# mwhoffman/pybo

Hardware: AMD Instinct MI355X
Metric: BO-step wall-clock (GP fit + 1e6-candidate acq sweep) at N obs; steps/sec (higher is better)
Workload: dtype f64

## Files before the change

pybo_amd/_lib.py:

```python
import ctypes as C
import os

import numpy as np



def hw_queues_hint():
    try:
        q = int(os.environ.get('GPU_MAX_HW_QUEUES', '4'))
    except ValueError:
        q = 4
    if q >= 8:
        return None
    return ('pybo_amd: several device handles on GPU_MAX_HW_QUEUES=%d hardware queues; export GPU_MAX_HW_QUEUES=8 before '
            'the HIP runtime starts to keep their streams apart (see INTEGRATION.md)' % q)


_HERE = os.path.dirname(os.path.abspath(__file__))
LIB_PATH = os.environ.get('GPX_LIB_PATH') or os.path.join(
    _HERE, 'csrc', 'libgpx_diag.so' if os.environ.get('GPX_DIAGNOSTICS', '0') not in ('', '0') else 'libgpx.so')

_P = C.c_void_p
_D = C.POINTER(C.c_double)
_I = C.POINTER(C.c_int64)
# ... 558 lines not shown
        ti = np.empty(k, dtype=np.int64)
        out = np.empty(M) if want_all else None
        mu = np.empty(M) if want_moments else None
        s2 = np.empty(M) if want_moments else None
        self._check(self._lib.gpx_sweep_update(self._h, aid, _ptr(params), nparams, k, _ptr(tv) if k else None,
                                               _ptr(ti) if k else None, _ptr(out), _ptr(mu), _ptr(s2)))
        return dict(top_val=tv, top_idx=ti, acq=out, mu=mu, s2=s2)

    def sweep_cache_size(self):
        return int(self._lib.gpx_sweep_cache_size(self._h))

    def sweep_batch(self, kind, param, nb, want_s2_all=False):
        aid = acq_id(kind)
        params, nparams = _acq_params(param)
        n = max(int(nb), 0)
        out = dict(sel_val=np.empty(n), sel_idx=np.empty(n, dtype=np.int64), sel_s2=np.empty(n))
        if want_s2_all:
            out['s2_all'] = np.empty(self.sweep_cache_size())
        self._check(self._lib.gpx_sweep_batch(self._h, aid, _ptr(params), nparams, int(nb), _ptr(out['sel_val']), _ptr(out['sel_idx']),
                                              _ptr(out['sel_s2']), _ptr(out.get('s2_all'))))
        return out

    def sweep_dev(self, acq, param, dXc_ptr, M, k, d_acq=None, d_mu=None, d_s2=None):
        aid = acq_id(acq)
        params, nparams = _acq_params(param)
        tv = np.empty(k)
        ti = np.empty(k, dtype=np.int64)
        self._check(self._lib.gpx_sweep_dev(self._h, aid, _ptr(params), nparams, _P(dXc_ptr), M, k,
                                            _ptr(tv) if k else None, _ptr(ti) if k else None,
                                            _P(d_acq) if d_acq else None, _P(d_mu) if d_mu else None,
                                            _P(d_s2) if d_s2 else None))
        return tv, ti

    @staticmethod
    def ensemble_sweep(engines, acq, param, Xc, k=0, want_all=True, want_moments=False):
        lead = engines[0]
        handles = (_P * len(engines))(*[e._h for e in engines])
        aid = acq_id(acq)
        params, nparams = _acq_params(param)
        tv = np.empty(k)
        ti = np.empty(k, dtype=np.int64)
        if isinstance(Xc, DeviceGrid):
            M = len(Xc)
            lead._check(lead._lib.gpx_ensemble_sweep_dev(handles, len(engines), aid, _ptr(params), nparams, Xc.ptr, M,
                                                         k, _ptr(tv) if k else None, _ptr(ti) if k else None,
                                                         None, None, None))
            return dict(top_val=tv, top_idx=ti, acq=None, mu=None, s2=None)
        Xc = _f64(Xc).reshape(-1, lead.d)
        M = len(Xc)
        out = np.empty(M) if want_all else None
        mu = np.empty(M) if want_moments else None
        s2 = np.empty(M) if want_moments else None
        lead._check(lead._lib.gpx_ensemble_sweep(handles, len(engines), aid, _ptr(params), nparams, _ptr(Xc), M, k,
                                                 _ptr(tv) if k else None, _ptr(ti) if k else None, _ptr(out),
                                                 _ptr(mu), _ptr(s2)))
        return dict(top_val=tv, top_idx=ti, acq=out, mu=mu, s2=s2)

    @staticmethod
    def ensemble_batch(engines, kind, param, nb):
        lead = engines[0]
        handles = (_P * len(engines))(*[e._h for e in engines])
        aid = acq_id(kind)
        params, nparams = _acq_params(param)
        n = max(int(nb), 0)
        out = dict(sel_val=np.empty(n), sel_idx=np.empty(n, dtype=np.int64), sel_s2=np.empty((len(engines), n)))
        lead._check(lead._lib.gpx_ensemble_sweep_batch(handles, len(engines), aid, _ptr(params), nparams, int(nb), _ptr(out['sel_val']),
                                                       _ptr(out['sel_idx']), _ptr(out['sel_s2'])))
        return out

    @staticmethod
    def ensemble_predict(engines, Xc):
        lead = engines[0]
        handles = (_P * len(engines))(*[e._h for e in engines])
        Xc = _f64(Xc).reshape(-1, lead.d)
        n, M, d = len(engines), len(Xc), lead.d
        mu, s2 = np.empty((n, M)), np.empty((n, M))
        dmu, ds2 = np.empty((n, M, d)), np.empty((n, M, d))
        lead._check(lead._lib.gpx_ensemble_predict(handles, n, _ptr(Xc), M, _ptr(mu), _ptr(s2), _ptr(dmu), _ptr(ds2)))
        return mu, s2, dmu, ds2

    def rff_gram(self, W, b):
        W = _f64(W)
        b = _f64(b)
        n = len(b)
        A = np.empty((n, n))
        v = np.empty(n)
        self._check(self._lib.gpx_rff_gram(self._h, _ptr(W), _ptr(b), n, _ptr(A), _ptr(v)))
        return A, v

    def rff_gram_batch(self, W, b):
        W = _f64(W)
        S, n, d = W.shape
        b = _f64(b).reshape(S, n)
        A = np.empty((S, n, n))
        v = np.empty((S, n))
        self._check(self._lib.gpx_rff_gram_batch(self._h, _ptr(W), _ptr(b), S, n, _ptr(A), _ptr(v)))
        return A, v

    def rff_posterior(self, W, b, z, sc):
        W = _f64(W)
        S, n, d = W.shape
        b = _f64(b).reshape(S, n)
        z = _f64(z).reshape(S, n)
        theta = np.empty((S, n))
        self._check(self._lib.gpx_rff_posterior(self._h, _ptr(W), _ptr(b), _ptr(z), S, n, float(sc), _ptr(theta)))
        return theta

    def rff_sweep(self, W, b, theta, bias, Xc, k=0, want_all=True):
        W = _f64(W)
        S, n, d = W.shape
        b = _f64(b).reshape(S, n)
        theta = _f64(theta).reshape(S, n)
        Xc = _f64(Xc).reshape(-1, d)
        M = len(Xc)
        tv = np.empty((S, k))
        ti = np.empty((S, k), dtype=np.int64)
        out = np.empty((S, M)) if want_all else None
        self._check(self._lib.gpx_rff_sweep(self._h, _ptr(W), _ptr(b), _ptr(theta), S, n, d, bias, _ptr(Xc), M,
                                            k, _ptr(tv) if k else None, _ptr(ti) if k else None, _ptr(out)))
        return dict(top_val=tv, top_idx=ti, vals=out)

    def rff_eval_grad(self, W, b, theta, bias, Xc):
        W = _f64(W)
        n, d = W.shape
        b = _f64(b)
        theta = _f64(theta)
        Xc = _f64(Xc).reshape(-1, d)
        M = len(Xc)
        f = np.empty(M)
        g = np.empty((M, d))
        self._check(self._lib.gpx_rff_grad(self._h, _ptr(W), _ptr(b), _ptr(theta), n, d, bias, _ptr(Xc), M,
                                           _ptr(f), _ptr(g)))
        return f, g

    def rff_sweep_dev(self, W, b, theta, bias, dXc_ptr, M, k):
        W = _f64(W)
        S, n, d = W.shape
        b = _f64(b).reshape(S, n)
        theta = _f64(theta).reshape(S, n)
        tv = np.empty((S, k))
        ti = np.empty((S, k), dtype=np.int64)
        self._check(self._lib.gpx_rff_sweep_dev(self._h, _ptr(W), _ptr(b), _ptr(theta), S, n, d, bias,
                                                _P(dXc_ptr), M, k, _ptr(tv), _ptr(ti), None))
        return tv, ti

    def timers(self, reset=False):
        out = np.zeros(len(TIMER_NAMES))
        self._lib.gpx_timers(self._h, _ptr(out), len(out), 1 if reset else 0)
        return dict(zip(TIMER_NAMES, out.tolist()))

    PRUNE_PATHS = ('plain', 'gate declined', 'pruned', 'fell back')

    def prune_report(self, vectors=True):
        scal = np.full(20, np.nan)
        self._check(self._lib.gpx_prune_report(self._h, _ptr(scal), len(scal), None, None, 0, None, None, 0))
        names = ('path', 'M', 'k', 'G', 'Gg', 'done', 'cap', 'nsurv', 'S', 'delta', 'tau', 'gate_s2', 'thr_key', 'kept',
                 'bound_kernel', 'guard', 'nR', 'nsurv2', 'E', 'gate_hint')
        r = dict(zip(names, scal.tolist()))
        r['gate_hint'] = r['gate_hint'] == 1.0
        r['bound_kernel'] = None if np.isnan(r['bound_kernel']) else ('generic', 'mfma', 'mfma32')[int(r['bound_kernel'])]
        for n in ('path', 'M', 'k', 'G', 'Gg', 'done', 'cap', 'nsurv', 'kept', 'nR', 'nsurv2'):
            r[n] = int(r[n])
        r['path'] = self.PRUNE_PATHS[r['path']]
        if vectors and r['path'] in ('pruned', 'fell back'):
            M = r['M']
            nidx = r['nsurv'] if r['path'] == 'pruned' else 0
            r['ub'] = np.empty(M)
            r['idx'] = np.empty(nidx, dtype=np.int64)
            kept = bool(r['kept'])
            r['ub_kept'] = np.empty(M) if kept else None
            r['seed_idx'] = np.empty(r['G'], dtype=np.int64) if kept else None
            self._check(self._lib.gpx_prune_report(self._h, _ptr(scal), len(scal), _ptr(r['ub']), _ptr(r['idx']), nidx,
                                                   _ptr(r['ub_kept']), _ptr(r['seed_idx']), r['G'] if kept else 0))
            if r['nR'] > 0 and kept:
                r['ub2'] = np.empty(nidx)
                r['idx2'] = np.empty(r['nsurv2'], dtype=np.int64)
                r['qR'] = np.empty(nidx)
                self._check(self._lib.gpx_prune_rows(self._h, _ptr(r['qR']), _ptr(r['ub2']), _ptr(r['idx2']), r['nsurv2']))
        return r

    @staticmethod
    def ensemble_prune_report(engines, vectors=True):
        lead = engines[0]
        handles = (_P * len(engines))(*[e._h for e in engines])
        scal = np.full(11 + len(engines), np.nan)
        lead._check(lead._lib.gpx_ensemble_prune_report(handles, len(engines), _ptr(scal), len(scal), None, None, 0))
        names = ('path', 'M', 'k', 'G', 'Gg', 'done', 'cap', 'nsurv', 'tau', 'gate')
        r = dict(zip(names, scal[:10].tolist()))
        for n in names[:8]:
            r[n] = int(r[n])
        r['path'] = Engine.PRUNE_PATHS[r['path']]
        r['delta'] = scal[10:10 + len(engines)].copy()
        r['gate_hint'] = scal[10 + len(engines)] == 1.0
        if vectors and r['path'] in ('pruned', 'fell back'):
            nidx = r['nsurv'] if r['path'] == 'pruned' else 0
            r['ub'] = np.empty(r['M'])
            r['idx'] = np.empty(nidx, dtype=np.int64)
            lead._check(lead._lib.gpx_ensemble_prune_report(handles, len(engines), _ptr(scal), len(scal), _ptr(r['ub']), _ptr(r['idx']),
                                                            nidx))
        return r

    def prune_dots(self):
        M = self.prune_report(vectors=False)['M']
        out = np.empty(M)
        self._check(self._lib.gpx_prune_dots(self._h, _ptr(out)))
        return out

    def chol_trace(self, nblocks, full_log=False):
        out = np.zeros(20 * nblocks + 8 * 1024 + 16 + (4 << 20 if full_log else 0), dtype=np.int64)
        n = self._lib.gpx_chol_trace(self._h, _ptr(out), out.size)
        if n < 20 * nblocks:
            return None
        self.last_chol_profile = out[20 * nblocks:20 * nblocks + 8192].reshape(1024, 8).copy()
        self.last_chol_tasklog = None
        if full_log and n >= out.size:
            self.last_chol_tasklog = out[20 * nblocks + 8192 + 16:].reshape(1024, 1024, 4).copy()
        out = out[:20 * nblocks]
        t0 = out[0]
        self.last_chol_trace_origin = int(t0)
        diag = (out[:4 * nblocks].reshape(nblocks, 4)[:, :3] - t0) / 100.0
        crit = out[4 * nblocks:].reshape(nblocks, 8, 2).astype(np.float64)
        crit = np.where(crit > 0, (crit - t0) / 100.0, np.nan)
        return diag, crit

    def sync(self):
        self._check(self._lib.gpx_sync(self._h))
```

pybo_amd/csrc/api.hip:

```cpp
#include <math.h>
#include <stdio.h>
#include <stdlib.h>
#include <string.h>

#include <algorithm>
#include <cmath>
#include <functional>
#include <new>

#include "gpx_internal.h"
#include "gpx_diag.h"
#include "mes_math.h"
#include "kg_math.h"

using namespace gpx;

static thread_local std::string g_create_err;

#define HIPCHK(h, call)                                                                     \
    do {                                                                                    \
        hipError_t e_ = (call);                                                             \
        if (e_ != hipSuccess) {                                                             \
            char buf_[512];                                                                 \
            snprintf(buf_, sizeof buf_, "%s failed: %s (%s:%d)", #call, hipGetErrorString(e_), \
                     __FILE__, __LINE__);                                                   \
            (h)->err = buf_;                                                                \
            return (e_ == hipErrorOutOfMemory) ? GPX_EOOM : GPX_EHIP;                       \
        }                                                                                   \
    } while (0)

static int fail(gpx_handle* h, int code, const char* msg) {
    h->err = msg;
    return code;
}

template <typename F>
static int guarded(gpx_handle* h, F&& body) noexcept {
    try {
        return body();
    } catch (const std::bad_alloc&) {
        if (h) {
            try { h->err = "out of host memory"; } catch (...) {}
        }
        return GPX_EOOM;
    } catch (...) {
        if (h) {
            try { h->err = "unexpected C++ exception inside libgpx"; } catch (...) {}
        }
        return GPX_EHIP;
    }
}

template <typename T>
static int ensure(gpx_handle* h, T*& p, int64_t& cap, int64_t need) {
    if (need <= cap && p) return GPX_OK;
    if (p) HIPCHK(h, hipFree(p));
    p = nullptr;
    cap = 0;
    HIPCHK(h, hipMalloc((void**)&p, (size_t)need * sizeof(T)));
    cap = need;
    return GPX_OK;
}

static hipEvent_t ev_get(gpx_handle* h) {
    if (!h->pool.empty()) {
        hipEvent_t e = h->pool.back();
        h->pool.pop_back();
        return e;
    }
    hipEvent_t e = nullptr;
    hipEventCreate(&e);
    return e;
}
static void harvest_finished(gpx_handle* h) {
    size_t keep = 0;
    for (size_t i = 0; i < h->pending.size(); ++i) {
        EventPair p = h->pending[i];
        if (hipEventQuery(p.b) == hipSuccess) {
            float ms = 0.f;
            if (hipEventElapsedTime(&ms, p.a, p.b) == hipSuccess) h->tacc[p.slot] += ms;
            h->pool.push_back(p.a);
            h->pool.push_back(p.b);
        } else {
            h->pending[keep++] = p;
        }
    }
    h->pending.resize(keep);
}

struct Span {
    gpx_handle* h;
    EventPair p;
    Span(gpx_handle* h_, int slot) : h(h_) {
        if (h->pending.size() >= 256) harvest_finished(h);
        p.a = ev_get(h);
        p.b = ev_get(h);
        p.slot = slot;
        hipEventRecord(p.a, h->stream);
    }
    ~Span() {
        hipEventRecord(p.b, h->stream);
        h->pending.push_back(p);
    }
};
static void harvest(gpx_handle* h) {
    hipStreamSynchronize(h->stream);
    if (h->spec_launched && h->stream3) hipStreamSynchronize(h->stream3);
    for (auto& p : h->pending) {
        float ms = 0.f;
        if (hipEventElapsedTime(&ms, p.a, p.b) == hipSuccess) h->tacc[p.slot] += ms;
        h->pool.push_back(p.a);
        h->pool.push_back(p.b);
    }
    h->pending.clear();
}

enum { SHIP = 0, DIAG = 1 };
struct Option {
    const char* name;
    int diag;
    int64_t lo, hi;
    const char* bad;
    void (*set)(gpx_handle* h, int64_t v);
    bool (*ok)(int64_t v) = nullptr;
    const char* bad_ok = nullptr;
};
template <int gpx_handle::*F>
static void store(gpx_handle* h, int64_t v) { h->*F = (int)v; }
static bool mult128(int64_t v) { return v % 128 == 0; }
static const int64_t BIG = INT64_MAX;
static const char* const TG = "chol_tg*: out of range";
static const char* const TRTRI = "trtri_ahead*: out of range";
static const char* const XBG = "x_bg*: out of range";
static const Option kOptions[] = {
    {"chunk", SHIP, 128, BIG, "chunk must be a positive multiple of 128", [](gpx_handle* h, int64_t v) { h->chunk = v; }, mult128},
    {"super_m", SHIP, 1, 16, "super_m must be 1, 2, 4, 8 or 16", store<&gpx_handle::super_m>, [](int64_t v) { return (v & (v - 1)) == 0; }},
    {"tile_order", SHIP, -1, 31, "tile_order: -1 (by size) or bits 0-1 tile map (0..3), bits 2-4 k-loop schedule (1 .. 7)",
     store<&gpx_handle::tile_order>, [](int64_t v) { return v == -1 || v >= 4; }},
    {"sweep_cache", SHIP, -1, 1, "sweep_cache must be 1, 0 or -1",
     [](gpx_handle* h, int64_t v) { h->cache_on = (v == 1); if (v < 0) { h->cache_valid = false; h->npend = 0; } }},
    {"prune", SHIP, -1, 1, "prune must be -1 (by size and gate), 0 (never) or 1 (wherever legal)", store<&gpx_handle::prune>},
    {"prune_keep", DIAG, 0, 1, "prune_keep must be 0 or 1", store<&gpx_handle::prune_keep>},
    {"prune_bound", DIAG, -1, 2, "prune_bound must be -1 (by guard), 0 (generic kernel), 1 (matrix-pipe kernel) or 2 (fp32 matrix-pipe kernel)", store<&gpx_handle::prune_bound>},
    {"prune_rows", DIAG, -1, 1000000, "prune_rows must be -1 (by size), 0 (no second bound) or a number of block rows", store<&gpx_handle::prune_rows>},
    {"short_map", DIAG, -1, 1, "short_map must be -1 (by size), 0 (never) or 1 (wherever tile map 3 is in use)", store<&gpx_handle::short_map>},
    {"chol_w", SHIP, 0, 8, "chol_w must be 0 (by size) or in [2, 8]", store<&gpx_handle::chol_w>, [](int64_t v) { return v != 1; }},
    {"chol_tg", SHIP, -1, 1000000000, TG, store<&gpx_handle::chol_tg>, [](int64_t v) { return v == 0 || v == 1; }, "chol_tg must be 0 or 1"},
    {"chol_tg_chunks", DIAG, -1, 1000000000, TG, store<&gpx_handle::tg_chunks>},
    {"chol_tg_grid", DIAG, -1, 1000000000, TG, store<&gpx_handle::tg_grid>},
    {"chol_tg_trace", DIAG, -1, 1000000000, TG, store<&gpx_handle::tg_trace>},
    {"chol_tg_isolate", DIAG, -1, 1000000000, TG, store<&gpx_handle::tg_isolate>},
    {"chol_tg_nap", DIAG, -1, 1000000000, TG, [](gpx_handle* h, int64_t v) { h->tg_nap = (int)std::max<int64_t>(0, std::min<int64_t>(127, v)); }},
    {"chol_tg_tmo_ms", SHIP, -1, 1000000000, TG, store<&gpx_handle::tg_tmo_ms>},
    {"chol_tg_min", SHIP, -1, 1000000000, TG, [](gpx_handle* h, int64_t v) { h->tg_min = (int)std::max<int64_t>(1, v); }},
    {"chol_tg_max", SHIP, -1, 1000000000, TG, [](gpx_handle* h, int64_t v) { h->tg_max = (int)std::max<int64_t>(1, v); }},
    {"chol_tg_db", SHIP, -1, 1000000000, TG, [](gpx_handle* h, int64_t v) { h->tg_db = (v < 0) ? -1 : (v != 0 ? 1 : 0); }},
    {"chol_tg_db_max", SHIP, -1, 1000000000, TG, [](gpx_handle* h, int64_t v) { h->tg_db_max = (int)std::max<int64_t>(0, v); }},
    {"chol_tg_fuse", SHIP, -1, 1000000000, TG, [](gpx_handle* h, int64_t v) { h->tg_fuse = (v != 0) ? 1 : 0; }},
    {"trtri_ahead", SHIP, 0, 1000000, TRTRI, [](gpx_handle* h, int64_t v) { h->trtri_ahead = (v != 0) ? 1 : 0; }},
    {"trtri_ahead_min", SHIP, 0, 1000000, TRTRI, [](gpx_handle* h, int64_t v) { h->trtri_ahead_min = (int)std::max<int64_t>(4, v); }},
    {"chol_fuse", SHIP, 0, 1, "chol_fuse must be 0 or 1", store<&gpx_handle::chol_fuse>},
    {"chol_graph", SHIP, 0, 1, "chol_graph must be 0 or 1", store<&gpx_handle::chol_graph>},
    {"chol_merge", SHIP, 0, 100000, "chol_merge: 0 (off) or a minimum number of block rows", store<&gpx_handle::chol_merge>},
    {"chol_rl", SHIP, 0, 1, "chol_rl must be 0 or 1", store<&gpx_handle::chol_rl>},
    {"x_skip", DIAG, 0, 7, "x_skip: bits 0..2", store<&gpx_handle::x_skip>},
    {"x_bg", DIAG, 0, 10000000, XBG, store<&gpx_handle::x_bg>},
    {"x_bg_lds", DIAG, 0, 10000000, XBG, store<&gpx_handle::x_bg_lds>},
    {"x_bg_iters", DIAG, 0, 10000000, XBG, store<&gpx_handle::x_bg_iters>},
    {"x_rff", DIAG, 0, 1, "x_rff must be 0 (by size) or 1 (the round-3 kernel)", [](gpx_handle*, int64_t v) { gpx::g_rff_variant = (int)v; }},
    {"grad_form", SHIP, 0, 2, "grad_form must be 0 (auto), 1 (two passes) or 2 (one pass)", store<&gpx_handle::grad_form>},
    {"grad_rb_cs", DIAG, 0, 65536, "grad_rb_cs must be a multiple of 128 (0 = default)", store<&gpx_handle::grad_rb_cs>, mult128},
    {"grad_kernel", SHIP, -1, 1, "grad_kernel must be -1 (auto), 0 or 1", store<&gpx_handle::grad_kernel>},
    {"trtri_left", SHIP, 0, 1, "trtri_left must be 0 or 1", store<&gpx_handle::trtri_left>},
    {"refine_inverse", SHIP, 0, 1, "refine_inverse must be 0 or 1", [](gpx_handle* h, int64_t v) { h->refine_inverse = (v != 0); }},
    {"eager_inverse", SHIP, 0, 1, "eager_inverse must be 0 or 1", [](gpx_handle* h, int64_t v) { h->eager_inverse = (v != 0); }},
};

extern "C" int gpx_set_option(gpx_handle* h, const char* name, int64_t value) {
    return guarded(h, [&]() -> int {
        if (!h) return GPX_EARG;
        h->prune_hint = h->ens_hint = PruneHint();
        if (!name) return GPX_EARG;
        for (const Option& o : kOptions) {
            if (strcmp(name, o.name)) continue;
            if (o.diag && !gpx_diagnostics())
                return fail(h, GPX_EARG, "diagnostic option: only in a library built with -DGPX_DIAGNOSTICS (libgpx_diag.so)");
            if (value < o.lo || value > o.hi) return fail(h, GPX_EARG, o.bad);
            if (o.ok && !o.ok(value)) return fail(h, GPX_EARG, o.bad_ok ? o.bad_ok : o.bad);
            o.set(h, value);
            return GPX_OK;
        }
        return fail(h, GPX_EARG, "unknown option");
    });
}

static std::string apply_env_options(gpx_handle* h) {
    const char* env = getenv("GPX_OPTIONS");
    const std::string all(env ? env : "");
    for (size_t pos = 0; pos < all.size();) {
        size_t end = all.find(',', pos);
        if (end == std::string::npos) end = all.size();
        const std::string kv = all.substr(pos, end - pos);
        pos = end + 1;
        if (kv.empty()) continue;
        const size_t eq = kv.find('=');
        char* tail = nullptr;
        const long long v = (eq == std::string::npos) ? 0 : strtoll(kv.c_str() + eq + 1, &tail, 10);
        if (eq == std::string::npos || eq == 0 || !tail || *tail != 0 || tail == kv.c_str() + eq + 1 ||
            gpx_set_option(h, kv.substr(0, eq).c_str(), (int64_t)v) != GPX_OK)
            return kv;
    }
    return "";
}

extern "C" int gpx_version(void) { return 680; }

extern "C" const char* gpx_last_error(const gpx_handle* h) {
    return h ? h->err.c_str() : g_create_err.c_str();
}

static int create_impl(int device, void* stream, gpx_handle** out);

extern "C" int gpx_create(int device, void* stream, gpx_handle** out) {
    try {
        return create_impl(device, stream, out);
    } catch (...) {
        if (out) *out = nullptr;
        return GPX_EOOM;
    }
}

static int create_impl(int device, void* stream, gpx_handle** out) {
    if (!out) { g_create_err = "gpx_create: out is NULL"; return GPX_EARG; }
    *out = nullptr;
    int ndev = 0;
    hipError_t e = hipGetDeviceCount(&ndev);
    if (e != hipSuccess || ndev <= 0) {
        g_create_err = std::string("gpx_create: no HIP device (") + hipGetErrorString(e) + ")";
        return GPX_EHIP;
    }
    if (device < 0 || device >= ndev) { g_create_err = "gpx_create: bad device index"; return GPX_EARG; }
    gpx_handle* h = new (std::nothrow) gpx_handle();
    if (!h) { g_create_err = "gpx_create: out of host memory"; return GPX_EOOM; }
    h->device = device;
    if ((e = hipSetDevice(device)) != hipSuccess) {
        g_create_err = std::string("hipSetDevice: ") + hipGetErrorString(e);
        delete h;
        return GPX_EHIP;
    }
    if (stream) {
        h->stream = (hipStream_t)stream;
    } else {
        if ((e = hipStreamCreateWithFlags(&h->stream, hipStreamNonBlocking)) != hipSuccess) {
            g_create_err = std::string("hipStreamCreate: ") + hipGetErrorString(e);
            delete h;
            return GPX_EHIP;
        }
        h->own_stream = true;
    }
    if (hipMalloc((void**)&h->dsmall, 64 + 16 * 8 + DMAX * 8 + 32) != hipSuccess) {
        g_create_err = "gpx_create: device allocation failed";
        delete h;
        return GPX_EOOM;
    }
    if (hipHostMalloc((void**)&h->hinv, (size_t)DMAX * 8, hipHostMallocDefault) != hipSuccess ||
        hipEventCreateWithFlags(&h->ev_inv, hipEventDisableTiming) != hipSuccess) {
        g_create_err = "gpx_create: pinned host allocation failed";
        hipFree(h->dsmall);
        delete h;
        return GPX_EOOM;
    }
    h->dflag = reinterpret_cast<int*>(h->dsmall);
    h->dscal = reinterpret_cast<double*>(h->dsmall + 64);
    h->dinvell = h->dscal + 16;
    h->dclk = reinterpret_cast<unsigned long long*>(h->dinvell + DMAX);
    (void)hipMemsetAsync(h->dclk, 0, 32, h->stream);
    (void)hipStreamSynchronize(h->stream);
    *out = h;
    const std::string bad = apply_env_options(h);
    if (!bad.empty()) {
        g_create_err = "gpx_create: GPX_OPTIONS: bad entry '" + bad + "'";
        *out = nullptr;
        gpx_destroy(h);
        return GPX_EARG;
    }
    return GPX_OK;
}

int gpx::ensure_side_streams(gpx_handle* h) {
    if (h->stream2) return GPX_OK;
    int prio_lo = 0, prio_hi = 0;
    hipDeviceGetStreamPriorityRange(&prio_lo, &prio_hi);
    bool ok_ev = true;
    for (auto& e : h->ev_row) ok_ev = ok_ev && hipEventCreateWithFlags(&e, hipEventDisableTiming) == hipSuccess;
    if (!ok_ev || hipStreamCreateWithPriority(&h->stream2, hipStreamNonBlocking, prio_lo) != hipSuccess ||
        hipStreamCreateWithFlags(&h->stream3, hipStreamNonBlocking) != hipSuccess ||
        hipStreamCreateWithPriority(&h->stream4, hipStreamNonBlocking, prio_lo) != hipSuccess ||
        hipEventCreateWithFlags(&h->ev_chain, hipEventDisableTiming) != hipSuccess ||
        hipEventCreateWithFlags(&h->ev_far, hipEventDisableTiming) != hipSuccess ||
        hipEventCreateWithFlags(&h->ev_rest, hipEventDisableTiming) != hipSuccess)
        return fail(h, GPX_EHIP, "side stream / event creation failed");
    return GPX_OK;
}

extern "C" int gpx_destroy(gpx_handle* h) {
    if (!h) return GPX_OK;
    hipSetDevice(h->device);
    hipStreamSynchronize(h->stream);
    if (h->ahead_top != 0 && h->stream2) { hipStreamSynchronize(h->stream2); h->ahead_top = 0; }
    tg_free(h);
    for (auto& p : h->pending) { hipEventDestroy(p.a); hipEventDestroy(p.b); }
    for (auto e : h->pool) hipEventDestroy(e);
    void* ptrs[] = {h->dXs, h->dXraw, h->dy, h->dS, h->dR, h->dT, h->dU, h->da, h->dalpha, h->dsmall, h->dKs, h->dQp, h->dXc, h->dout, h->dblkv, h->dblki,
                    h->dtopv, h->drff, h->drffs, h->dgrad, h->dens, h->dprune, h->dkeep, h->dcZ, h->dcq, h->dbatch, h->dhyper, h->dpend, h->drefine, h->dspec, h->dbsel, h->djoint, h->dkg, h->dkgw};
    for (void* p : ptrs)
        if (p) hipFree(p);
    if (h->hpin) hipHostFree(h->hpin);
    if (h->hinv) hipHostFree(h->hinv);
    if (h->chol_exec) hipGraphExecDestroy(h->chol_exec);
    if (h->ev_inv) hipEventDestroy(h->ev_inv);
    if (h->ev_spec_go) hipEventDestroy(h->ev_spec_go);
    if (h->ev_spec_done) hipEventDestroy(h->ev_spec_done);
    if (h->stream_bg) { hipStreamSynchronize(h->stream_bg); hipStreamDestroy(h->stream_bg); }
    if (h->stream2) { hipStreamSynchronize(h->stream2); hipStreamDestroy(h->stream2); }
    if (h->stream3) { hipStreamSynchronize(h->stream3); hipStreamDestroy(h->stream3); }
    if (h->stream4) { hipStreamSynchronize(h->stream4); hipStreamDestroy(h->stream4); }
    if (h->ev_rest) hipEventDestroy(h->ev_rest);
    for (auto e : h->ev_row)
        if (e) hipEventDestroy(e);
    if (h->ev_chain) hipEventDestroy(h->ev_chain);
    if (h->ev_far) hipEventDestroy(h->ev_far);
    if (h->own_stream) hipStreamDestroy(h->stream);
    delete h;
    return GPX_OK;
}


extern "C" int gpx_sync(gpx_handle* h) {
    return guarded(h, [&]() -> int {
        if (!h) return GPX_EARG;
        HIPCHK(h, hipStreamSynchronize(h->stream));
        return GPX_OK;
    });
}

extern "C" int64_t gpx_chol_tasks2(int nblocks, int chunks, int16_t* out, int64_t cap, int64_t* counts) {
    if (!counts) return -1;
    try {
        return gpx::tg_tasks_copy(nblocks, chunks, out, cap, counts);
    } catch (...) {
        return -1;
    }
}

extern "C" int64_t gpx_chol_trace(gpx_handle* h, int64_t* out, int64_t n) {
    if (!h || !out || n <= 0) return 0;
    if (hipSetDevice(h->device) != hipSuccess || hipStreamSynchronize(h->stream) != hipSuccess) return 0;
    static_assert(sizeof(long long) == sizeof(int64_t), "trace words");
    return tg_trace_copy(h, reinterpret_cast<long long*>(out), n);
}

static void report_head(const gpx_handle::SelectRecord& r, double* out) {
    const double head[8] = {(double)r.path, (double)r.M, (double)r.k, (double)r.G, (double)r.Gg, (double)r.done, (double)r.cap, (double)r.nsurv};
    std::copy(head, head + 8, out);
}
static int report_vectors(gpx_handle* h, const gpx_handle::SelectRecord& r, double* ub, int64_t* idx, int64_t cap_idx) {
    if (ub) HIPCHK(h, hipMemcpy(ub, r.ub, (size_t)r.M * 8, hipMemcpyDeviceToHost));
    const int64_t nidx = std::min(std::min(r.nsurv, r.cap), cap_idx);
    if (idx && nidx > 0) HIPCHK(h, hipMemcpy(idx, r.idx, (size_t)nidx * 8, hipMemcpyDeviceToHost));
    return GPX_OK;
}

extern "C" int gpx_prune_report(gpx_handle* h, double* scal, int nscal, double* ub, int64_t* idx, int64_t cap_idx,
                                double* ub_kept, int64_t* seed_idx, int64_t cap_seed) {
    return guarded(h, [&]() -> int {
        if (!h) return GPX_EARG;
        if (!scal || nscal < 0) return fail(h, GPX_EARG, "prune_report: NULL output");
        const gpx_handle::PruneRecord& r = h->prune_rec;
        if (r.path < 0) return fail(h, GPX_ESTATE, "prune_report: no sweep has completed its argument checks since the record was last cleared");
        const bool bound = r.path >= 2;
        if ((ub || idx || ub_kept || seed_idx) && !bound)
            return fail(h, GPX_ESTATE, "prune_report: the last sweep did not reach its bound pass");
        if ((ub_kept || seed_idx) && !r.kept)
            return fail(h, GPX_ESTATE, "prune_report: the last sweep ran without the option prune_keep");
        HIPCHK(h, hipSetDevice(h->device));
        HIPCHK(h, hipStreamSynchronize(h->stream));
        double sc[16];
        int st[4] = {0, 0, 0, 0};
        for (double& v : sc) v = NAN;
        if (bound) {
            HIPCHK(h, hipMemcpy(sc, r.sc, sizeof sc, hipMemcpyDeviceToHost));
            HIPCHK(h, hipMemcpy(st, r.st, sizeof st, hipMemcpyDeviceToHost));
        }
        const bool guarded_bound = bound && r.bound_kernel < 0;
        double out[20];
        report_head(r, out);
        const double tail[12] = {sc[0], sc[1], sc[5], r.gate, bound ? (double)st[2] : NAN, r.kept ? 1.0 : 0.0,
                                 bound ? (guarded_bound ? sc[9] + sc[12] : 0.0) : NAN, guarded_bound ? sc[8] : NAN,
                                 (double)r.nR, (double)r.nsurv2, guarded_bound ? sc[10] : NAN, r.hinted ? 1.0 : 0.0};
        std::copy(tail, tail + 12, out + 8);
        for (int i = 0; i < nscal && i < 20; ++i) scal[i] = out[i];
        int rc;
        if ((rc = report_vectors(h, r, ub, idx, cap_idx))) return rc;
        if (ub_kept) HIPCHK(h, hipMemcpy(ub_kept, h->dkeep, (size_t)r.M * 8, hipMemcpyDeviceToHost));
        const int64_t nseed = std::min(r.G, cap_seed);
        if (seed_idx && nseed > 0)
            HIPCHK(h, hipMemcpy(seed_idx, h->dkeep + r.M * 8, (size_t)nseed * 8, hipMemcpyDeviceToHost));
        return GPX_OK;
    });
}

extern "C" int gpx_prune_rows(gpx_handle* h, double* qR, double* ub2, int64_t* idx2, int64_t cap_idx2) {
    return guarded(h, [&]() -> int {
        if (!h) return GPX_EARG;
        const gpx_handle::PruneRecord& r = h->prune_rec;
        if (r.path != 2 || r.nR <= 0) return fail(h, GPX_ESTATE, "prune_rows: the last sweep ran no second bound");
        if (!r.kept) return fail(h, GPX_ESTATE, "prune_rows: the last sweep ran without the option prune_keep");
        HIPCHK(h, hipSetDevice(h->device));
        HIPCHK(h, hipStreamSynchronize(h->stream));
        if (qR) HIPCHK(h, hipMemcpy(qR, r.qR, (size_t)r.nsurv * 8, hipMemcpyDeviceToHost));
        if (ub2) HIPCHK(h, hipMemcpy(ub2, r.ub2, (size_t)r.nsurv * 8, hipMemcpyDeviceToHost));
        const int64_t n2 = std::min(r.nsurv2, cap_idx2);
        if (idx2 && n2 > 0) HIPCHK(h, hipMemcpy(idx2, r.idx2, (size_t)n2 * 8, hipMemcpyDeviceToHost));
        return GPX_OK;
    });
}

extern "C" int gpx_prune_dots(gpx_handle* h, double* dots) {
    return guarded(h, [&]() -> int {
        if (!h) return GPX_EARG;
        if (!dots) return fail(h, GPX_EARG, "prune_dots: NULL output");
        const gpx_handle::PruneRecord& r = h->prune_rec;
        if (r.path < 2 || !r.kept) return fail(h, GPX_ESTATE, "prune_dots: the last sweep kept no bound pass (option prune_keep)");
        HIPCHK(h, hipSetDevice(h->device));
        HIPCHK(h, hipStreamSynchronize(h->stream));
        HIPCHK(h, hipMemcpy(dots, h->dkeep + (r.M + r.G) * 8, (size_t)r.M * 8, hipMemcpyDeviceToHost));
        return GPX_OK;
    });
}

extern "C" int gpx_timers(gpx_handle* h, double* out, int n, int reset) {
    return guarded(h, [&]() -> int {
        if (!h) return GPX_EARG;
        if (!out || n < 0) return fail(h, GPX_EARG, "timers: NULL output");
        harvest(h);
        unsigned long long clk[4] = {0, 0, 0, 0};
        (void)hipMemcpyAsync(clk, h->dclk, 32, hipMemcpyDeviceToHost, h->stream);
        (void)hipStreamSynchronize(h->stream);
        h->tacc[T_SCLK] = clk[1] ? 100.0 * (double)clk[0] / (double)clk[1] : 0.0;
        h->tacc[T_RFFCLK] = clk[3] ? 100.0 * (double)clk[2] / (double)clk[3] : 0.0;
        const int m = std::min(n, (int)T_COUNT);
        for (int i = 0; i < m; ++i) out[i] = h->tacc[i];
        if (reset) {
            for (int i = 0; i < T_COUNT; ++i) h->tacc[i] = 0;
            (void)hipMemsetAsync(h->dclk, 0, 32, h->stream);
        }
        return m;
    });
}

static void spec_cancel(gpx_handle* h) {
    if (h->spec_launched && h->ev_spec_done) hipStreamWaitEvent(h->stream, h->ev_spec_done, 0);
    h->spec_active = false;
    h->spec_launched = false;
    h->apply_pending = false;
}

static int check_fit_args(gpx_handle* h, const void* X, int64_t N, int64_t d, const void* y, int kid,
                          const double* ell, double rho, double sn2) {
    if (!h) return GPX_EARG;
    if (!X || !y || !ell) return fail(h, GPX_EARG, "fit: NULL pointer");
    if (N < 1) return fail(h, GPX_EARG, "fit: N must be >= 1");
    if (d < 1 || d > DMAX) return fail(h, GPX_EARG, "fit: d must be in [1, 1024]");
    if (kid < GPX_KERN_SE_ARD || kid > GPX_KERN_MATERN12) return fail(h, GPX_EARG, "fit: unknown kernel id");
    if (!(rho > 0) || !(sn2 >= 0) || !std::isfinite(rho) || !std::isfinite(sn2))
        return fail(h, GPX_EARG, "fit: need finite rho > 0 and sn2 >= 0");
    for (int64_t k = 0; k < d; ++k)
        if (!(ell[k] > 0) || !std::isfinite(ell[k]))
            return fail(h, GPX_EARG, "fit: length-scales must be positive and finite");
    return GPX_OK;
}

static int alloc_model(gpx_handle* h, int64_t Np, int64_t d) {
    if (Np > h->cap_np || d > h->cap_d) {
        Np = std::max(Np + std::max<int64_t>(NB, Np / 16 / NB * NB), h->cap_np);
        d = std::max(d, h->cap_d);
        double** mats[] = {&h->dS, &h->dR, &h->dT, &h->dU};
        for (auto m : mats) {
            if (*m) HIPCHK(h, hipFree(*m));
            *m = nullptr;
        }
        double** vecs[] = {&h->dy, &h->da, &h->dalpha, &h->dXs, &h->dXraw};
        for (auto v : vecs) {
            if (*v) HIPCHK(h, hipFree(*v));
            *v = nullptr;
        }
        h->cap_np = 0;
        h->cap_d = 0;
        for (auto m : mats) {
            HIPCHK(h, hipMalloc((void**)m, (size_t)Np * Np * 8));
            HIPCHK(h, hipMemsetAsync(*m, 0, (size_t)Np * Np * 8, h->stream));
        }
        HIPCHK(h, hipMalloc((void**)&h->dy, (size_t)Np * 8));
        HIPCHK(h, hipMalloc((void**)&h->da, (size_t)Np * 8));
        HIPCHK(h, hipMalloc((void**)&h->dalpha, (size_t)Np * 8));
        HIPCHK(h, hipMalloc((void**)&h->dXs, (size_t)Np * d * 8));
        HIPCHK(h, hipMalloc((void**)&h->dXraw, (size_t)Np * d * 8));
        h->cap_np = Np;
        h->cap_d = d;
    }
    return GPX_OK;
}

static void settle_ahead(gpx_handle* h) {
    if (h->ahead_top == 0) return;
    (void)hipStreamSynchronize(h->stream2);
    h->ahead_top = 0;
}

int gpx::ensure_inverse(gpx_handle* h) {
    if (h->stage >= 3) return GPX_OK;
    if (h->stage < 2) return fail(h, GPX_ESTATE, "model is not fitted");
    HIPCHK(h, hipSetDevice(h->device));
    {
        Span sp(h, T_TRTRI);
        launch_trtri(h);
        if (h->refine_inverse) {
            int rc = ensure(h, h->drefine, h->cap_refine, h->cap_np * h->cap_np);
            if (rc) return rc;
            launch_refine_inverse(h, h->drefine);
        }
    }
    {
        Span sp(h, T_ALPHA);
        launch_alpha(h);
    }
    HIPCHK(h, hipGetLastError());
    h->stage = 3;
    return GPX_OK;
}

static int fit_core(gpx_handle* h, const double* dX, int64_t N, int64_t d, const double* dy, int kid,
                    const double* ell, double rho, double sn2, double bias, int stage) {
    HIPCHK(h, hipSetDevice(h->device));
    const int64_t Np = (N + NB - 1) / NB * NB;
    spec_cancel(h);
    settle_ahead(h);
    const bool prev_inverse_used = h->stage >= 3;
    ++h->gen;
    h->fitted = false;
    h->stage = 0;
    h->fail_pivot = -1;
    h->last_topn = 0;
    h->cache_valid = false;
// ... 360 lines not shown
    {
        Span sp(h, T_ACQ);
        launch_topk(s, d_vals, M, (int)k, h->dblkv, h->dblki, nblk, h->dtopv, h->dtopi);
    }
    h->last_topv = h->dtopv; h->last_topi = h->dtopi; h->last_topn = k;
    HIPCHK(h, hipMemcpyAsync(top_val, h->dtopv, (size_t)k * 8, hipMemcpyDeviceToHost, s));
    HIPCHK(h, hipMemcpyAsync(top_idx, h->dtopi, (size_t)k * 8, hipMemcpyDeviceToHost, s));
    HIPCHK(h, hipStreamSynchronize(s));
    return GPX_OK;
}

struct AcqRule { int id, min_params; bool vec; };
static const AcqRule ACQ_RULES[] = {
    {GPX_ACQ_EI, 1, false}, {GPX_ACQ_PI, 1, false}, {GPX_ACQ_UCB, 1, false}, {GPX_ACQ_MEAN, 0, false}, {GPX_ACQ_MES, 1, true},
};
static int check_acq(gpx_handle* h, const char* what, int acq_id, const double* params, int nparams, int n_members = 0, bool kg_ok = false) {
    if (acq_id == GPX_ACQ_KG) {
        if (!kg_ok) return fail(h, GPX_EARG, (std::string(what) + ": KG is not supported").c_str());
        bool ok = params && h->d > 0 && nparams >= h->d && nparams % h->d == 0 && nparams / h->d <= KG_MAX_M;
        for (int i = 0; ok && i < nparams; ++i) ok = std::isfinite(params[i]);
        if (!ok) return fail(h, GPX_EARG, (std::string(what) + ": KG takes m * d finite support coordinates, m in [1, 127]").c_str());
        return GPX_OK;
    }
    const AcqRule* rule = nullptr;
    for (const AcqRule& r : ACQ_RULES)
        if (r.id == acq_id) rule = &r;
    if (!rule) return fail(h, GPX_EARG, (std::string(what) + ": unknown acquisition id").c_str());
    if (rule->vec) {
        if (n_members > 0 && (!params || nparams < n_members || nparams % n_members != 0 || nparams / n_members > MES_MAX_S))
            return fail(h, GPX_EARG, (std::string(what) + ": MES takes n_members * S maximum samples, S in [1, 64]").c_str());
        bool ok = params && nparams >= 1 && (n_members > 0 || nparams <= MES_MAX_S);
        for (int i = 0; ok && i < nparams; ++i) ok = std::isfinite(params[i]);
        if (!ok) return fail(h, GPX_EARG, (std::string(what) + ": MES takes 1 to 64 finite maximum samples").c_str());
        return GPX_OK;
    }
    if (rule->min_params > 0 && (nparams < rule->min_params || !params))
        return fail(h, GPX_EARG, (std::string(what) + ": missing acquisition parameter").c_str());
    return GPX_OK;
}
static int check_acq_batch(gpx_handle* h, const char* what, int acq_id) {
    if (acq_id == GPX_ACQ_MES) return fail(h, GPX_EARG, (std::string(what) + ": MES is not supported").c_str());
    if (acq_id == GPX_ACQ_KG) return fail(h, GPX_EARG, (std::string(what) + ": KG is not supported").c_str());
    return GPX_OK;
}
static MesArg mes_arg(const double* params, int nparams) {
    MesArg a;
    a.S = nparams;
    for (int i = 0; i < MES_MAX_S; ++i) a.y[i] = i < nparams ? params[i] : 0.0;
    return a;
}

struct KgBuf { double *A, *As, *al, *B, *V, *Pp; int m; };
static KgBuf kg_layout(const gpx_handle* h, int m) {
    KgBuf b;
    b.A = h->dkg;
    b.As = b.A + NB * h->d;
    b.al = b.As + NB * h->d;
    b.B = b.al + NB;
    b.V = b.B + h->Np * NB;
    b.Pp = b.V + h->Np * NB;
    b.m = m;
    return b;
}
static int kg_prepare(gpx_handle* h, const double* A, int m, KgBuf& b) {
    const int64_t Np = h->Np, d = h->d;
    const int nP = (int)(Np / NB);
    const int64_t need = 2 * NB * d + NB + 2 * Np * NB + (int64_t)nP * NB;
    if (need > h->cap_kg || !h->dkg) h->kg_A.clear();
    int rc;
    if ((rc = ensure(h, h->dkg, h->cap_kg, need))) return rc;
    if ((rc = ensure(h, h->dKs, h->cap_ks, Np * NB))) return rc;
    b = kg_layout(h, m);
    const size_t na = (size_t)m * d;
    if (h->kg_gen == h->gen && h->kg_Np == Np && h->kg_A.size() == na && memcmp(h->kg_A.data(), A, na * 8) == 0) return GPX_OK;
    h->kg_A.clear();
    hipStream_t s = h->stream;
    {
        Span sp(h, T_COPY);
        HIPCHK(h, hipMemcpyAsync(b.A, A, na * 8, hipMemcpyHostToDevice, s));
    }
    {
        Span sp(h, T_ACQ);
        launch_scale_x(s, b.A, m, NB, (int)d, h->dinvell, b.As);
        launch_cross_gram(s, h->dXs, Np, h->N, (int)d, b.A, 0, m, NB, h->dinvell, h->kernel_id, h->rho, h->dKs, Np);
        launch_cov_trmm(s, h->dU, Np, h->dKs, NB, b.V);
        launch_cov_mu(s, b.V, Np, NB, h->da, h->bias, b.Pp, b.al);
        launch_kg_solve(s, h->dU, Np, h->N, m, b.V, b.B);
        HIPCHK(h, hipGetLastError());
    }
    h->kg_A.assign(A, A + na);
    h->kg_gen = h->gen;
    h->kg_Np = Np;
    return GPX_OK;
}

static int check_topk(gpx_handle* h, const char* what, int64_t k, const double* top_val, const int64_t* top_idx) {
    if (k < 0 || k > TOPK_MAX) return fail(h, GPX_EARG, (std::string(what) + ": k must be in [0, 4096]").c_str());
    if (k > 0 && (!top_val || !top_idx)) return fail(h, GPX_EARG, (std::string(what) + ": NULL top-k output").c_str());
    return GPX_OK;
}

template <typename Core>
static int staged_sweep(gpx_handle* h, const double* Xc, int64_t M, bool sync_upload, double* acq_all, double* mu, double* s2,
                        Core&& core) {
    HIPCHK(h, hipSetDevice(h->device));
    const int64_t nx = Xc ? M * h->d : 0;
    int rc;
    if ((rc = ensure(h, h->dXc, h->cap_xc, nx + 3 * M))) return rc;
    double* dX = h->dXc;
    double* dacq = dX + nx;
    double* dmu = dacq + M;
    double* ds2 = dmu + M;
    if (Xc) {
        Span sp(h, T_COPY);
        HIPCHK(h, hipMemcpyAsync(dX, Xc, (size_t)nx * 8, hipMemcpyHostToDevice, h->stream));
    }
    if (sync_upload) HIPCHK(h, hipStreamSynchronize(h->stream));
    if ((rc = core(dX, acq_all ? dacq : nullptr, mu ? dmu : nullptr, s2 ? ds2 : nullptr))) return rc;
    {
        Span sp(h, T_COPY);
        if (acq_all) HIPCHK(h, hipMemcpyAsync(acq_all, dacq, (size_t)M * 8, hipMemcpyDeviceToHost, h->stream));
        if (mu) HIPCHK(h, hipMemcpyAsync(mu, dmu, (size_t)M * 8, hipMemcpyDeviceToHost, h->stream));
        if (s2) HIPCHK(h, hipMemcpyAsync(s2, ds2, (size_t)M * 8, hipMemcpyDeviceToHost, h->stream));
    }
    HIPCHK(h, hipStreamSynchronize(h->stream));
    return GPX_OK;
}

static const int64_t PRUNE_MIN_M = 32768, PRUNE_MIN_NP = 1024, PRUNE_MAX_SHARE_DIV = 4;
static const double PRUNE_GATE_S2 = 1.0 / 64.0;
static const int PRUNE_ROWS_MIN_NP = 32, PRUNE_ROWS_DIV = 4;

struct PruneGeom { int64_t G, Gg, cap; };
static PruneGeom prune_geom(int nP, int64_t k, int64_t M) {
    const int64_t gen_tiles = std::max<int64_t>(1, 512 / ((nP + 1) / 2));
    const int64_t G0 = (int64_t)TBH * std::min<int64_t>(32, gen_tiles);
    const int64_t G = std::max<int64_t>(G0, (k + TBH - 1) / TBH * TBH);
    return {G, (int64_t)TBH * gen_tiles, std::max<int64_t>(G, M / PRUNE_MAX_SHARE_DIV)};
}

struct PruneWs {
    double *ub, *vals, *Xg;
    int64_t *idx, *blk;
    double *alpha2, *sabs, *gs2, *sc, *extra;
    int *hist, *st;
    double* bws;
    int64_t nsel;
    double *dots, *ub2, *qR, *Xg2;
    int64_t *idx2, *blk2;
};
static int prune_ws(gpx_handle* h, int64_t M, int64_t cap, int64_t Gg, int64_t extra, PruneWs& w, bool rows = false) {
    const int64_t Np = h->Np;
    w.nsel = sel_blocks(M);
    const int64_t words0 = M + cap + cap * h->d + cap + (w.nsel + 1) + 2 * Np + Gg + 16 + extra + (2 * 4096 + 8) / 2;
    const int64_t words1 = (words0 + 3) / 4 * 4 + bound_mfma_ws_words(Np);
    const int64_t words = words1 + (rows ? M + 3 * cap + cap * h->d + sel_blocks(cap) + 1 : 0);
    if (!h->dprune || words * 8 > h->cap_prune) h->ens_rec = gpx_handle::EnsPruneRecord();
    int rc;
    if ((rc = ensure(h, h->dprune, h->cap_prune, words * 8))) return rc;
    w.ub = reinterpret_cast<double*>(h->dprune);
    w.vals = w.ub + M;
    w.Xg = w.vals + cap;
    w.idx = reinterpret_cast<int64_t*>(w.Xg + cap * h->d);
    w.blk = w.idx + cap;
    w.alpha2 = reinterpret_cast<double*>(w.blk + w.nsel + 1);
    w.sabs = w.alpha2 + Np;
    w.gs2 = w.sabs + Np;
    w.sc = w.gs2 + Gg;
    w.extra = w.sc + 16;
    w.hist = reinterpret_cast<int*>(w.extra + extra);
    w.st = w.hist + 2 * 4096;
    w.bws = w.ub + (words0 + 3) / 4 * 4;
    w.dots = w.ub2 = w.qR = w.Xg2 = nullptr;
    w.idx2 = w.blk2 = nullptr;
    if (!rows) return GPX_OK;
    w.dots = w.ub + words1;
    w.ub2 = w.dots + M;
    w.qR = w.ub2 + cap;
    w.idx2 = reinterpret_cast<int64_t*>(w.qR + cap);
    w.Xg2 = reinterpret_cast<double*>(w.idx2 + cap);
    w.blk2 = reinterpret_cast<int64_t*>(w.Xg2 + cap * h->d);
    return GPX_OK;
}

static const int64_t BOUND_F32_MIN_M = 131072;
static void bound_dots(gpx_handle* h, const double* dXc, int64_t M, const PruneWs& w, bool bound_mfma, double* out) {
    hipStream_t s = h->stream;
    launch_prune_alpha(s, h->dU, h->Np, h->da, h->rho, h->bias, w.alpha2, w.sabs, w.sc);
    if (bound_mfma)
        launch_bound_mfma(s, h->dXs, h->N, h->Np, (int)h->d, w.alpha2, h->rho, dXc, M, h->dinvell, h->prune_bound, M >= BOUND_F32_MIN_M, w.bws,
                          w.sc, out);
    launch_sweep_rank1_v(s, h->dXs, h->N, (int)h->d, w.alpha2, h->Np, w.sc + 2, dXc, M, h->dinvell, h->kernel_id, h->rho,
                         nullptr, out, bound_mfma ? w.sc + 9 : nullptr);
}

static int64_t sweep_chunk(const gpx_handle* h, int64_t M) {
    const int64_t chunk_opt = h->chunk > 0 ? h->chunk : (h->Np <= 4096 ? 131072 : 65536);
    return std::min<int64_t>(chunk_opt, (M + TBH - 1) / TBH * TBH);
}

struct SelectList { const double* X; int64_t* idx; int64_t n; };
struct SelectOps {
    std::function<int(const double* X, int64_t mb, int64_t me, double* out, double* mu, double* s2)> exact;
    std::function<int(int64_t Gg, double* value, bool* go)> gate;
    std::function<int(double* ub, int64_t done)> bound;
    std::function<int()> after_seeds;
    std::function<int(SelectList& list)> refine;
};

template <typename Rec>
static int select_topk_pruned(gpx_handle* L, bool legal, bool selection_only, int acq_id, int n, int nP, int64_t Np_min, const double* dXc,
                              int64_t M, int64_t k, int64_t ws_extra, bool ws_rows, PruneWs& w, PruneHint& hint, Rec& rec, double* out,
                              const SelectOps& ops, int64_t* done) {
    const PruneGeom geom = prune_geom(nP, k, M);
    const int64_t G = geom.G, Gg = geom.Gg, cap = geom.cap;
    const Rec fresh = rec;
    auto start_rec = [&]() {
        rec = fresh;
        rec.path = 0, rec.M = M, rec.k = k, rec.G = G, rec.Gg = Gg, rec.cap = cap, rec.gate = NAN;
    };
    start_rec();
    *done = 0;
    legal = legal && selection_only && acq_id == GPX_ACQ_EI && k > 0 && L->prune != 0 && M >= 3 * G;
    bool pruning = legal && (L->prune == 1 || (M >= PRUNE_MIN_M && Np_min >= PRUNE_MIN_NP && M >= Gg + 2 * G));
    if (!pruning) return GPX_OK;
    hipStream_t s = L->stream;
    int rc;
    const int64_t kk = std::min<int64_t>(k, TOPK_PASS);
    if ((rc = ensure(L, L->dblkv, L->cap_blk, topk_blocks(M) * kk))) return rc;
    if ((rc = ensure(L, L->dblki, L->cap_blki, topk_blocks(M) * kk))) return rc;
    if ((rc = ensure(L, L->dtopv, L->cap_top, (int64_t)TOPK_MAX * 2))) return rc;
    L->dtopi = reinterpret_cast<int64_t*>(L->dtopv + TOPK_MAX);
    if ((rc = prune_ws(L, M, cap, Gg, ws_extra, w, ws_rows))) return rc;
    start_rec();
    PruneHint key;
    key.kernel_id = L->kernel_id, key.n = n, key.d = L->d, key.nP = nP, key.Np_min = Np_min, key.M = M, key.k = k;
    const bool automatic = L->prune < 0;
    if (automatic && prune_hint_matches(hint, key)) {
        rec.hinted = true;
    } else if (automatic) {
        if ((rc = ops.gate(Gg, &rec.gate, &pruning))) return rc;
        *done = Gg;
        rec.path = 1;
    }
    if (automatic) hint = PruneHint();
    if (!pruning) return GPX_OK;
    double *const ub = w.ub, *const vals = w.vals, *const Xg = w.Xg;
    if ((rc = ops.bound(ub, *done))) return rc;
    {
        Span sp(L, T_ACQ);
        launch_sel_threshold(s, ub, M, (int)G, w.hist, w.st);
        launch_sel_compact(s, ub, M, 0, w.st, nullptr, w.blk, G, dXc, (int)L->d, w.idx, Xg);
    }
    if (ops.after_seeds && (rc = ops.after_seeds())) return rc;
    if ((rc = ops.exact(Xg, 0, G, vals, nullptr, nullptr))) return rc;
    int64_t nsurv = 0;
    {
        Span sp(L, T_ACQ);
        launch_topk(s, vals, G, (int)k, L->dblkv, L->dblki, topk_blocks(G), L->dtopv, L->dtopi);
        launch_fill_neg_inf(s, out, *done, M);
        launch_sel_scatter(s, w.idx, vals, G, out, ub);
        launch_sel_compact(s, ub, M, 1, w.st, L->dtopv + (k - 1), w.blk, cap, dXc, (int)L->d, w.idx, Xg, w.sc + 5);
        HIPCHK(L, hipMemcpyAsync(&nsurv, w.blk + w.nsel, 8, hipMemcpyDeviceToHost, s));
    }
    HIPCHK(L, hipStreamSynchronize(s));
    rec.path = nsurv <= cap ? 2 : 3, rec.done = *done, rec.nsurv = nsurv;
    rec.ub = ub, rec.idx = w.idx, rec.sc = w.sc;
    if (automatic) hint = key, hint.armed = prune_hint_after(rec.path, nsurv, cap);
    if (nsurv > cap) return GPX_OK;
    SelectList list = {Xg, w.idx, nsurv};
    if (ops.refine && (rc = ops.refine(list))) return rc;
    if (list.n > 0) {
        if ((rc = ops.exact(list.X, 0, list.n, vals, nullptr, nullptr))) return rc;
        Span sp(L, T_ACQ);
        if (list.idx != w.idx) launch_sel_remap(s, w.idx, list.idx, list.n);
        launch_sel_scatter(s, list.idx, vals, list.n, out, nullptr);
    }
    *done = M;
    return GPX_OK;
}

static int plain_rest(const SelectOps& ops, const double* dXc, int64_t done, int64_t chunk, int64_t M, double* out, double* mu, double* s2) {
    const int64_t chunk1 = std::min(chunk, M);
    int rc;
    if (done > 0 && done < chunk1) {
        if ((rc = ops.exact(dXc, done, chunk1, out, mu, s2))) return rc;
        done = chunk1;
    }
    return done < M ? ops.exact(dXc, done, M, out, mu, s2) : GPX_OK;
}

static int second_bound(gpx_handle* h, const PruneWs& w, int64_t chunk, int sweep_order, double p0, SelectList& list) {
    hipStream_t s = h->stream;
    gpx_handle::PruneRecord& rec = h->prune_rec;
    const int64_t Np = h->Np, M = rec.M, Gg = rec.Gg, cap = rec.cap, nsurv = list.n;
    const int nP = (int)(Np / NB);
    int nR = 0;
    if (h->prune_rows > 0) nR = (int)std::min<int64_t>(std::min<int64_t>(h->prune_rows, nP), h->N / NB);
    else if (h->prune_rows < 0 && M >= PRUNE_MIN_M && nP >= PRUNE_ROWS_MIN_NP && nsurv > Gg) nR = std::max(1, nP / PRUNE_ROWS_DIV);
    if (nR <= 0 || nsurv <= 0) return GPX_OK;
    int64_t nsurv2 = 0;
    {
        Span sp(h, T_BOUND);
        for (int64_t j0 = 0; j0 < nsurv; j0 += chunk) {
            const int64_t valid = std::min(chunk, nsurv - j0);
            const int64_t cols = (valid + TBH - 1) / TBH * TBH;
            launch_cross_gram(s, h->dXs, (int64_t)nR * NB, h->N, (int)h->d, w.Xg, j0, nsurv, cols, h->dinvell, h->kernel_id, h->rho, h->dKs, Np);
            launch_sweep_trmm(s, h->dU, Np, nR, h->dKs, chunk, cols, h->da, h->dQp, h->dPp, chunk, sweep_order, h->super_m, h->dclk, h->short_map);
            launch_prune_ub2(s, h->dQp, chunk, nR, j0, valid, w.idx, w.dots, w.sc, h->rho, h->bias, p0, w.ub2, h->prune_keep ? w.qR : nullptr);
        }
    }
    {
        Span sp(h, T_ACQ);
        launch_sel_compact(s, w.ub2, nsurv, 1, w.st, w.sc + 5, w.blk2, cap, w.Xg, (int)h->d, w.idx2, w.Xg2);
        HIPCHK(h, hipMemcpyAsync(&nsurv2, w.blk2 + sel_blocks(nsurv), 8, hipMemcpyDeviceToHost, s));
    }
    HIPCHK(h, hipStreamSynchronize(s));
    rec.nR = nR, rec.nsurv2 = nsurv2;
    rec.ub2 = w.ub2, rec.idx2 = w.idx2, rec.qR = h->prune_keep ? w.qR : nullptr;
    list = {w.Xg2, w.idx2, nsurv2};
    return GPX_OK;
}

static int sweep_core(gpx_handle* h, int acq_id, const double* params, int nparams, const double* dXc,
                      int64_t M, int64_t k, double* top_val, int64_t* top_idx, double* d_acq,
                      double* d_mu, double* d_s2) {
    h->prune_rec = gpx_handle::PruneRecord();
    if (!h->fitted) return fail(h, GPX_ESTATE, "sweep: model is not fitted");
    if (!dXc || M < 1) return fail(h, GPX_EARG, "sweep: need M >= 1 candidates");
    int rc;
    if ((rc = check_acq(h, "sweep", acq_id, params, nparams, 0, true)) || (rc = check_topk(h, "sweep", k, top_val, top_idx))) return rc;
    HIPCHK(h, hipSetDevice(h->device));
    if ((rc = ensure_inverse(h))) return rc;
    hipStream_t s = h->stream;
    const int64_t Np = h->Np;
    const int nP = (int)(Np / NB);
    const int64_t chunk = sweep_chunk(h, M);
    if ((rc = ensure(h, h->dKs, h->cap_ks, Np * chunk))) return rc;
    if ((rc = ensure(h, h->dQp, h->cap_part, (int64_t)nP * chunk * 2))) return rc;
    h->dPp = h->dQp + (int64_t)nP * chunk;
    const bool selection_only = !d_acq && !d_mu && !d_s2;
    if (!d_acq) {
        if ((rc = ensure(h, h->dout, h->cap_out, M))) return rc;
        d_acq = h->dout;
// ... 637 lines not shown
            HIPCHK(h, hipSetDevice(h->device));
            hipStream_t s = h->stream;
            const int64_t d = h->d, Np = h->Np, N = h->N, np = (n + NB - 1) / NB * NB;
            int rc;
            const int64_t need = n * d + 6 * n + n * n + 2 * np * np + n * Np;
            if ((rc = ensure(h, h->drff, h->cap_rff, need))) return rc;
            double* dW = h->drff;
            double* db = dW + n * d;
            double* dA = db + n;
            double* dv = dA + n * n;
            double* dz = dv + n;
            double* dwork = dz + n;
            double* dth = dwork + n;
            double* dB = dth + n;
            double* dR = dB + np * np;
            double* dFt = dR + np * np;
            int* pflag = h->dflag + 8;
            for (int64_t q = 0; q < S; ++q) {
                if ((rc = upload_draw(h, W, b, q, n, dW, db))) return rc;
                HIPCHK(h, hipMemcpyAsync(dz, z + q * n, (size_t)n * 8, hipMemcpyHostToDevice, s));
                int flag = 0;
                {
                    Span sp(h, T_RFF);
                    launch_rff_gram(s, h->dXraw, dFt, N, (int)d, dW, db, (int)n, h->dy, h->bias, dA, dv);
                    launch_posterior_wide(s, dA, dv, dz, (int)n, np, sc, h->sn2, dB, dR, dwork, pflag, dth);
                }
                HIPCHK(h, hipMemcpyAsync(theta + q * n, dth, (size_t)n * 8, hipMemcpyDeviceToHost, s));
                HIPCHK(h, hipMemcpyAsync(&flag, pflag, sizeof(int), hipMemcpyDeviceToHost, s));
                HIPCHK(h, hipStreamSynchronize(s));
                HIPCHK(h, hipGetLastError());
                if (flag != 0) return fail(h, GPX_ENOTPD, "rff_posterior: the feature Gram of a draw is not positive definite");
            }
            return GPX_OK;
        }
        HIPCHK(h, hipSetDevice(h->device));
        hipStream_t s = h->stream;
        int rc;
        double *dA, *dv, *dz;
        if ((rc = rff_gram_batch_dev(h, W, b, S, n, 2 * S * n, &dA, &dv, &dz))) return rc;
        double* dth = dz + S * n;
        int* pflag = h->dflag + 8;
        HIPCHK(h, hipMemsetAsync(pflag, 0, sizeof(int), s));
        HIPCHK(h, hipMemcpyAsync(dz, z, (size_t)S * n * 8, hipMemcpyHostToDevice, s));
        {
            Span sp(h, T_RFF);
            launch_rff_posterior(s, dA, dv, dz, (int)S, (int)n, sc, h->sn2, dth, pflag);
        }
        int flag = 0;
        HIPCHK(h, hipMemcpyAsync(theta, dth, (size_t)S * n * 8, hipMemcpyDeviceToHost, s));
        HIPCHK(h, hipMemcpyAsync(&flag, pflag, sizeof(int), hipMemcpyDeviceToHost, s));
        HIPCHK(h, hipStreamSynchronize(s));
        HIPCHK(h, hipGetLastError());
        if (flag != 0) return fail(h, GPX_ENOTPD, "rff_posterior: the feature Gram of a draw is not positive definite");
        return GPX_OK;
    });
}

extern "C" int gpx_rff_gram(gpx_handle* h, const double* W, const double* b, int64_t n, double* A, double* v) {
    return guarded(h, [&]() -> int {
        return gpx_rff_gram_batch(h, W, b, 1, n, A, v);
    });
}

static int member_fail(gpx_handle* L, const gpx_handle* h, int m, int rc) {
    if (h != L) L->err = "ensemble member " + std::to_string(m) + ": " + h->err;
    return rc;
}

static int ensemble_core(gpx_handle* const* mem, int n, int acq_id, const double* params, int nparams,
                         const double* dXc, int64_t M, int64_t k, double* top_val, int64_t* top_idx,
                         double* d_out, double* d_mu, double* d_s2) {
    gpx_handle* L = mem[0];
    L->ens_rec = gpx_handle::EnsPruneRecord();
    int rc;
    if ((rc = check_acq(L, "ensemble_sweep", acq_id, params, nparams, n))) return rc;
    const int mesS = (acq_id == GPX_ACQ_MES) ? nparams / n : 0;
    if (!dXc || M < 1) return fail(L, GPX_EARG, "ensemble_sweep: need M >= 1 candidates");
    if ((rc = check_topk(L, "ensemble_sweep", k, top_val, top_idx))) return rc;
    for (int m = 0; m < n; ++m) {
        if (!mem[m]->fitted) return fail(L, GPX_ESTATE, "ensemble_sweep: a member model is not fitted");
        if (mem[m]->device != L->device || mem[m]->d != L->d)
            return fail(L, GPX_EARG, "ensemble_sweep: members must share the device and the input dimension");
    }
    HIPCHK(L, hipSetDevice(L->device));
    const int mode = (acq_id == GPX_ACQ_UCB || acq_id == GPX_ACQ_MEAN) ? 1 : 0;
    if ((rc = ensure(L, L->dens, L->cap_ens, 5 * M))) return rc;
    double* acc0 = L->dens;
    double* acc1 = acc0 + M;
    double* t0 = acc1 + M;
    double* t1 = t0 + M;
    double* out = d_out ? d_out : t1 + M;
    const double beta = (acq_id == GPX_ACQ_UCB) ? params[0] : 0.0;

    auto members = [&](const double* X, int64_t cnt, double* o, double* o_mu, double* o_s2, double* gate_mean) -> int {
        for (int m = 0; m < n; ++m) {
            gpx_handle* h = mem[m];
            int rcm = (mode == 0) ? sweep_core(h, acq_id, mesS ? params + (size_t)m * mesS : params, mesS ? mesS : nparams, X, cnt, 0, nullptr,
                                               nullptr, t0, nullptr, gate_mean ? t1 : nullptr)
                                  : sweep_core(h, GPX_ACQ_MEAN, nullptr, 0, X, cnt, 0, nullptr, nullptr, nullptr, t0, t1);
            if (rcm) return member_fail(L, h, m, rcm);
            if (gate_mean) launch_prune_mean(h->stream, t1, cnt, gate_mean + m);
            HIPCHK(L, hipStreamSynchronize(h->stream));
            launch_ens_accum(L->stream, acc0, acc1, t0, t1, cnt, mode, m == 0);
            HIPCHK(L, hipStreamSynchronize(L->stream));
        }
        if (acq_id == GPX_ACQ_MEAN)
            launch_ens_finish(L->stream, acc0, acc1, cnt, 1, (double)n, 0.0, o, o_mu, o_s2);
        else
            launch_ens_finish(L->stream, acc0, acc1, cnt, mode, (double)n, beta, o, o_mu, o_s2);
        return GPX_OK;
    };

    int nPmax = 0;
    int64_t Np_min = INT64_MAX;
    bool members_ok = true;
    for (int m = 0; m < n; ++m) {
        nPmax = std::max(nPmax, (int)(mem[m]->Np / NB));
        Np_min = std::min(Np_min, mem[m]->Np);
        members_ok = members_ok && !mem[m]->cache_on && mem[m]->rho >= 1e-100 && mem[m]->rho < INFINITY;
    }
    const int64_t d = L->d;
    hipStream_t s = L->stream;
    gpx_handle::EnsPruneRecord& rec = L->ens_rec;
    rec.n = n;
    PruneWs w;
    SelectOps ops;
    ops.exact = [&](const double* X, int64_t mb, int64_t me, double* o, double* o_mu, double* o_s2) -> int {
        return members(X + mb * d, me - mb, o + mb, o_mu ? o_mu + mb : nullptr, o_s2 ? o_s2 + mb : nullptr, nullptr);
    };
    ops.gate = [&](int64_t Gg, double* value, bool* go) -> int {
        if ((rc = members(dXc, Gg, out, nullptr, nullptr, w.extra))) return rc;
        std::vector<double> gm((size_t)n);
        HIPCHK(L, hipMemcpyAsync(gm.data(), w.extra, (size_t)n * 8, hipMemcpyDeviceToHost, s));
        HIPCHK(L, hipStreamSynchronize(s));
        double g = 0.0;
        for (int m = 0; m < n; ++m) g += gm[m] / mem[m]->rho;
        *value = g / (double)n;
        *go = *value >= PRUNE_GATE_S2;
        return GPX_OK;
    };
    ops.bound = [&](double* ub, int64_t done) -> int {
        double* const delta = w.extra + n;
        for (int m = 0; m < n; ++m) {
            gpx_handle* h = mem[m];
            HIPCHK(L, hipSetDevice(h->device));
            if ((rc = ensure_inverse(h))) return member_fail(L, h, m, rc);
            PruneWs wm = w;
            if (h != L) {
                h->prune_rec = gpx_handle::PruneRecord();
                if ((rc = prune_ws(h, 0, 0, 0, 0, wm))) return member_fail(L, h, m, rc);
            }
            {
                Span sp(h, T_BOUND);
                bound_dots(h, dXc, M, wm, h->prune_bound != 0 && bound_mfma_ks(h->kernel_id, (int)h->d) > 0, t1);
                launch_prune_ub_fold(h->stream, t1, ub, M, wm.sc, h->rho, h->bias, params[0], m == 0, delta + m);
            }
            HIPCHK(L, hipStreamSynchronize(h->stream));
        }
        {
            Span sp(L, T_BOUND);
            launch_prune_ub_mean(s, ub, M, done, (double)n);
        }
        rec.delta = delta;
        return GPX_OK;
    };
    ops.after_seeds = [&]() -> int { HIPCHK(L, hipStreamSynchronize(s)); return GPX_OK; };
    int64_t done = 0;
    if ((rc = select_topk_pruned(L, members_ok, !d_out && !d_mu && !d_s2, acq_id, n, nPmax, Np_min, dXc, M, k, 2 * n, false, w, L->ens_hint, rec,
                                 out, ops, &done)))
        return rc;
    if ((rc = plain_rest(ops, dXc, done, sweep_chunk(L, M), M, out, d_mu, d_s2))) return rc;
    if (k > 0) {
        if ((rc = topk_core(L, out, M, k, top_val, top_idx))) return rc;
    } else {
        HIPCHK(L, hipStreamSynchronize(L->stream));
    }
    HIPCHK(L, hipGetLastError());
    return GPX_OK;
}

static int ensemble_check(gpx_handle* const* members, int n) {
    if (!members || n < 1 || !members[0]) return GPX_EARG;
    for (int m = 1; m < n; ++m)
        if (!members[m]) {
            members[0]->err = "ensemble_sweep: NULL member handle";
            return GPX_EARG;
        }
    return GPX_OK;
}

extern "C" int gpx_ensemble_predict(gpx_handle* const* members, int n_members, const double* Xc, int64_t M,
                                    double* mu, double* s2, double* dmu, double* ds2) {
    if (ensemble_check(members, n_members)) return GPX_EARG;
    gpx_handle* h = members[0];
    return guarded(h, [&]() -> int {
        if (!mu || !s2 || !dmu || !ds2) return fail(h, GPX_EARG, "ensemble_predict: all four outputs are required");
        return gpx::ensemble_predict_grad_host(members, n_members, Xc, M, mu, s2, dmu, ds2);
    });
}

extern "C" int gpx_ensemble_sweep_dev(gpx_handle* const* members, int n_members, int acq_id, const double* params,
                                      int nparams, const double* dXc, int64_t M, int64_t k, double* top_val,
                                      int64_t* top_idx, double* d_acq_all, double* d_mu, double* d_s2) {
    if (ensemble_check(members, n_members)) return GPX_EARG;
    return guarded(members[0], [&]() -> int {
        return ensemble_core(members, n_members, acq_id, params, nparams, dXc, M, k, top_val, top_idx, d_acq_all,
                             d_mu, d_s2);
    });
}

extern "C" int gpx_ensemble_sweep(gpx_handle* const* members, int n_members, int acq_id, const double* params,
                                  int nparams, const double* Xc, int64_t M, int64_t k, double* top_val,
                                  int64_t* top_idx, double* acq_all, double* mu, double* s2) {
    if (ensemble_check(members, n_members)) return GPX_EARG;
    gpx_handle* h = members[0];
    return guarded(h, [&]() -> int {
        h->ens_rec = gpx_handle::EnsPruneRecord();
        if (!Xc || M < 1) return fail(h, GPX_EARG, "ensemble_sweep: need M >= 1 candidates");
        if ((mu || s2) && acq_id != GPX_ACQ_UCB && acq_id != GPX_ACQ_MEAN)
            return fail(h, GPX_EARG, "ensemble_sweep: mixture moments are only formed for UCB / mean");
        return staged_sweep(h, Xc, M, true, acq_all, mu, s2, [&](double* dX, double* dacq, double* dmu, double* ds2) {
            return ensemble_core(members, n_members, acq_id, params, nparams, dX, M, k, top_val, top_idx, dacq, dmu, ds2);
        });
    });
}

extern "C" int gpx_ensemble_sweep_batch(gpx_handle* const* members, int n_members, int acq_id, const double* params,
                                        int nparams, int64_t nb, double* sel_val, int64_t* sel_idx, double* sel_s2) {
    if (members && members[0] && (n_members < 1 || n_members > 64)) {
        members[0]->err = "ensemble_sweep_batch: n_members must be in [1, 64]";
        return GPX_EARG;
    }
    if (ensemble_check(members, n_members)) return GPX_EARG;
    gpx_handle* L = members[0];
    return guarded(L, [&]() -> int {
        const int n = n_members;
        int rc;
        if ((rc = check_acq_batch(L, "ensemble_sweep_batch", acq_id)) || (rc = check_acq(L, "ensemble_sweep_batch", acq_id, params, nparams)))
            return rc;
        if (acq_id == GPX_ACQ_MEAN)
            return fail(L, GPX_EARG, "ensemble_sweep_batch: the posterior mean does not change under hallucinated observations (EI, PI or UCB)");
        if (nb < 1 || nb > 64) return fail(L, GPX_EARG, "ensemble_sweep_batch: nb must be in [1, 64]");
        if (!sel_val || !sel_idx) return fail(L, GPX_EARG, "ensemble_sweep_batch: NULL sel_val / sel_idx output");
        for (int m = 0; m < n; ++m) {
            if (!members[m]->fitted) return fail(L, GPX_ESTATE, "ensemble_sweep_batch: a member model is not fitted");
            if (members[m]->device != L->device || members[m]->d != L->d)
                return fail(L, GPX_EARG, "ensemble_sweep_batch: members must share the device and the input dimension");
            for (int o = 0; o < m; ++o)
                if (members[o] == members[m])
                    return fail(L, GPX_EARG, "ensemble_sweep_batch: a handle is listed twice (every member needs its own scratch)");
        }
        for (int m = 0; m < n; ++m)
            if (!members[m]->cache_valid)
                return fail(L, GPX_ESTATE, ("ensemble member " + std::to_string(m) + ": ensemble_sweep_batch: no live sweep cache (sweep with "
                                            "option sweep_cache = 1 first)").c_str());
        const int64_t M = L->cache_M, d = L->d;
        for (int m = 1; m < n; ++m)
            if (members[m]->cache_M != M) return fail(L, GPX_EARG, "ensemble_sweep_batch: the members' caches differ in size");
        if (nb > M) return fail(L, GPX_EARG, "ensemble_sweep_batch: nb exceeds the number of cached candidates");
        HIPCHK(L, hipSetDevice(L->device));
        const int64_t desc_words = ((int64_t)n * (int64_t)sizeof(EnsBatchMember) + 7) / 8;
        std::vector<BatchBuf> bufs((size_t)n);
        L->bsel_desc.assign((size_t)n, EnsBatchMember());
        for (int m = 0; m < n; ++m) {
            gpx_handle* h = members[m];
            if ((rc = ensure_inverse(h)) || (rc = flush_pending(h)) ||
                (rc = batch_layout(h, M, nb, m == 0 ? (int64_t)n * nb + desc_words : 0, bufs[m]))) {
                if (h != L) L->err = "ensemble member " + std::to_string(m) + ": " + h->err;
                return rc;
            }
            HIPCHK(L, hipStreamSynchronize(h->stream));
            const BatchBuf& b = bufs[m];
            EnsBatchMember& e = L->bsel_desc[m];
            e.cq = h->dcq, e.cp = h->dcp, e.invell = h->dinvell;
            e.qp = b.qp, e.V = b.V, e.cross = b.cross, e.scal = b.scal, e.xs = b.xs;
            e.rho = h->rho, e.bias = h->bias, e.sn2 = h->sn2;
        }
        const BatchBuf& lb = bufs[0];
        double* dsel_s2 = lb.extra;
        EnsBatchMember* ddesc = reinterpret_cast<EnsBatchMember*>(lb.extra + (int64_t)n * nb);
        const double p0 = params[0];
        hipStream_t s = L->stream;
        int differ = 0;
        {
            Span sp(L, T_BATCH);
            HIPCHK(L, hipMemcpyAsync(ddesc, L->bsel_desc.data(), (size_t)n * sizeof(EnsBatchMember), hipMemcpyHostToDevice, s));
            HIPCHK(L, hipMemsetAsync(lb.taken, 0, (size_t)lb.ntaken * 8, s));
            HIPCHK(L, hipMemsetAsync(lb.same, 0, sizeof(int), s));
            for (int m = 0; m < n; ++m) {
                HIPCHK(L, hipMemsetAsync(bufs[m].flag, 0, sizeof(int), s));
                if (m > 0) launch_ens_same_grid(s, L->dcZ, members[m]->dcZ, M * d, lb.same);
            }
            for (int j = 0; j < (int)nb; ++j) {
                launch_ens_batch_score(s, j - 1, n, M, ddesc, lb.taken, acq_id, p0, lb.partv, lb.parti);
                launch_ens_batch_pick(s, j, n, nb, M, (int)d, lb.partv, lb.parti, L->dcZ, ddesc, lb.x, lb.sel_val, lb.sel_idx,
                                      dsel_s2, lb.taken);
                if (j == (int)nb - 1) break;
                for (int m = 0; m < n; ++m) batch_condition(members[m], s, bufs[m], lb.x, L->dcZ, M, j);
            }
            HIPCHK(L, hipGetLastError());
        }
        HIPCHK(L, hipMemcpyAsync(sel_val, lb.sel_val, (size_t)nb * 8, hipMemcpyDeviceToHost, s));
        HIPCHK(L, hipMemcpyAsync(sel_idx, lb.sel_idx, (size_t)nb * 8, hipMemcpyDeviceToHost, s));
        if (sel_s2) HIPCHK(L, hipMemcpyAsync(sel_s2, dsel_s2, (size_t)n * nb * 8, hipMemcpyDeviceToHost, s));
        HIPCHK(L, hipMemcpyAsync(&differ, lb.same, sizeof(int), hipMemcpyDeviceToHost, s));
        HIPCHK(L, hipStreamSynchronize(s));
        if (differ) return fail(L, GPX_EARG, "ensemble_sweep_batch: the members' caches hold different candidates");
        return GPX_OK;
    });
}

extern "C" int gpx_ensemble_prune_report(gpx_handle* const* members, int n_members, double* scal, int nscal, double* ub,
                                         int64_t* idx, int64_t cap_idx) {
    if (ensemble_check(members, n_members)) return GPX_EARG;
    gpx_handle* h = members[0];
    return guarded(h, [&]() -> int {
        if (!scal || nscal < 0) return fail(h, GPX_EARG, "ensemble_prune_report: NULL output");
        const gpx_handle::EnsPruneRecord& r = h->ens_rec;
        if (r.path < 0 || r.n != n_members)
            return fail(h, GPX_ESTATE, "ensemble_prune_report: no ensemble sweep of these members has completed its argument checks "
                                       "since the record was last cleared");
        const bool bound = r.path >= 2;
        if ((ub || idx) && !bound) return fail(h, GPX_ESTATE, "ensemble_prune_report: the last ensemble sweep did not reach its bound pass");
        HIPCHK(h, hipSetDevice(h->device));
        HIPCHK(h, hipStreamSynchronize(h->stream));
        std::vector<double> out((size_t)(11 + n_members), NAN);
        out[10 + n_members] = r.hinted ? 1.0 : 0.0;
        report_head(r, out.data());
        out[9] = r.gate;
        if (bound) {
            HIPCHK(h, hipMemcpy(&out[8], r.sc + 5, 8, hipMemcpyDeviceToHost));
            HIPCHK(h, hipMemcpy(&out[10], r.delta, (size_t)n_members * 8, hipMemcpyDeviceToHost));
        }
        for (int i = 0; i < nscal && i < 11 + n_members; ++i) scal[i] = out[i];
        return report_vectors(h, r, ub, idx, cap_idx);
    });
}

struct gpx_grid {
    int device = 0;
    int64_t M = 0, d = 0;
    double* dX = nullptr;
    hipStream_t s = nullptr;
};

#define GRIDCHK(call)                                                                              \
    do {                                                                                           \
        hipError_t e_ = (call);                                                                    \
        if (e_ != hipSuccess) {                                                                    \
            g_create_err = std::string(#call) + " failed: " + hipGetErrorString(e_);               \
            return (e_ == hipErrorOutOfMemory) ? GPX_EOOM : GPX_EHIP;                              \
        }                                                                                          \
    } while (0)

static int grid_create_impl(int device, int kind, const double* bounds, int64_t M, int64_t d, uint64_t seed,
                            int64_t first, const uint32_t* sv, int bits, gpx_grid** out) {
    if (!out) return GPX_EARG;
    *out = nullptr;
    if (!bounds || M < 1 || d < 1 || d > DMAX) { g_create_err = "grid_create: bad sizes or NULL bounds"; return GPX_EARG; }
    if (kind != GPX_GRID_UNIFORM && kind != GPX_GRID_SOBOL) { g_create_err = "grid_create: unknown grid kind"; return GPX_EARG; }
    if (first < 0) { g_create_err = "grid_create: first must be >= 0"; return GPX_EARG; }
    if (kind == GPX_GRID_SOBOL && (!sv || bits < 1 || bits > 32 || first < 0 ||
                                   (bits < 63 && (uint64_t)(first + M) > (1ull << bits)))) {
        g_create_err = "grid_create: Sobol needs direction numbers (d, bits), 1 <= bits <= 32, first + M <= 2^bits";
        return GPX_EARG;
    }
    GRIDCHK(hipSetDevice(device));
    gpx_grid* g = new gpx_grid();
    g->device = device; g->M = M; g->d = d;
    double* dB = nullptr;
    uint32_t* dsv = nullptr;
    auto cleanup = [&]() { if (dB) hipFree(dB); if (dsv) hipFree(dsv); };
    auto bail = [&](int rc) { cleanup(); if (g->dX) hipFree(g->dX); if (g->s) hipStreamDestroy(g->s); delete g; return rc; };
#define GRIDTRY(call)                                                                              \
    do {                                                                                           \
        hipError_t e_ = (call);                                                                    \
        if (e_ != hipSuccess) {                                                                    \
            g_create_err = std::string(#call) + " failed: " + hipGetErrorString(e_);               \
            return bail((e_ == hipErrorOutOfMemory) ? GPX_EOOM : GPX_EHIP);                        \
        }                                                                                          \
    } while (0)
    GRIDTRY(hipStreamCreateWithFlags(&g->s, hipStreamNonBlocking));
    GRIDTRY(hipMalloc((void**)&g->dX, (size_t)M * d * 8));
    GRIDTRY(hipMalloc((void**)&dB, (size_t)d * 2 * 8));
    GRIDTRY(hipMemcpyAsync(dB, bounds, (size_t)d * 2 * 8, hipMemcpyHostToDevice, g->s));
    if (kind == GPX_GRID_SOBOL) {
        GRIDTRY(hipMalloc((void**)&dsv, (size_t)d * bits * 4));
        GRIDTRY(hipMemcpyAsync(dsv, sv, (size_t)d * bits * 4, hipMemcpyHostToDevice, g->s));
        launch_grid_sobol(g->s, dsv, bits, first, M, (int)d, dB, g->dX);
    } else {
        launch_grid_uniform(g->s, seed, first, M, (int)d, dB, g->dX);
    }
    GRIDTRY(hipGetLastError());
    GRIDTRY(hipStreamSynchronize(g->s));
    cleanup();
    *out = g;
    return GPX_OK;
}

extern "C" int gpx_grid_create(int device, int kind, const double* bounds, int64_t M, int64_t d, uint64_t seed,
                               int64_t first, const uint32_t* sv, int bits, gpx_grid** out) {
    try {
        return grid_create_impl(device, kind, bounds, M, d, seed, first, sv, bits, out);
    } catch (...) {
        if (out) *out = nullptr;
        return GPX_EOOM;
    }
}

extern "C" const double* gpx_grid_data(const gpx_grid* g) { return g ? g->dX : nullptr; }

extern "C" int gpx_grid_rows(gpx_grid* g, const int64_t* idx, int64_t k, double* out) {
    try {
        if (!g || !out) { g_create_err = "grid_rows: NULL pointer"; return GPX_EARG; }
        GRIDCHK(hipSetDevice(g->device));
        if (!idx) {
            GRIDCHK(hipMemcpyAsync(out, g->dX, (size_t)g->M * g->d * 8, hipMemcpyDeviceToHost, g->s));
            GRIDCHK(hipStreamSynchronize(g->s));
            return GPX_OK;
        }
        if (k < 1) return GPX_OK;
        for (int64_t i = 0; i < k; ++i)
            if (idx[i] < 0 || idx[i] >= g->M) { g_create_err = "grid_rows: index out of range"; return GPX_EARG; }
        for (int64_t i = 0; i < k;) {
            int64_t j = i + 1;
            while (j < k && idx[j] == idx[j - 1] + 1) ++j;
            GRIDCHK(hipMemcpyAsync(out + i * g->d, g->dX + idx[i] * g->d, (size_t)(j - i) * g->d * 8, hipMemcpyDeviceToHost, g->s));
            i = j;
        }
        GRIDCHK(hipStreamSynchronize(g->s));
        return GPX_OK;
    } catch (...) {
        return GPX_EOOM;
    }
}

extern "C" int gpx_grid_destroy(gpx_grid* g) {
    if (!g) return GPX_OK;
    hipSetDevice(g->device);
    if (g->dX) hipFree(g->dX);
    if (g->s) hipStreamDestroy(g->s);
    delete g;
    return GPX_OK;
}
```

pybo_amd/csrc/bound_f32.h:

```cpp
#ifndef GPX_BOUND_F32_H
#define GPX_BOUND_F32_H

#include <cmath>

#if defined(__HIPCC__) || defined(__CUDACC__)
#define GPX_B32_FN __host__ __device__ __forceinline__
#else
#define GPX_B32_FN inline
#endif

namespace gpx {

constexpr double B32_U = 0x1p-24;
constexpr double B32_UX = 0x1p-22;
constexpr double B32_LOG2E = 1.44269504088896340736;
constexpr double B32_E_MAX = 0x1p-10;
constexpr double B32_W_MIN = 0x1p-126, B32_W_MAX = 0x1.fffffep+127;

GPX_B32_FN double bound32_bad_weight(double w) {
    const double a = std::fabs(w);
    return (a == 0.0 || (a >= B32_W_MIN && a <= B32_W_MAX)) ? 0.0 : 1.0;
}

GPX_B32_FN double bound32_E(int d, double depth, double gv) {
    const double eps_e = 0.5 * B32_LOG2E * (double)(d + 5) * (gv / (double)(d + 4)) * B32_U;
    const double eta = std::exp2(eps_e) * (1.0 + B32_UX) * (1.0 + B32_U) - 1.0;
    const double nu = depth * B32_U;
    if (!(nu < 0.5) || !(eta < 1.0)) return HUGE_VAL;
    const double g = nu / (1.0 - nu) + 0x1p-48;
    return (g * (1.0 + eta) + eta) * (1.0 + 0x1p-8);
}

GPX_B32_FN double bound32_factor(double E, double bad_weight) { return (E < 0.5 && bad_weight == 0.0) ? E / (1.0 - E) : HUGE_VAL; }

GPX_B32_FN double bound32_flush(double sum_w, double Np) { return 0x1p-124 * (sum_w + Np); }

GPX_B32_FN double bound32_hi(double A, double B, double factor, double F) {
    if (!(factor < HUGE_VAL)) return (A != A || B != B) ? A + B : HUGE_VAL;
    const double m = factor * B + F;
    return std::fma(0x1p-50, std::fabs(A) + m, A + m);
}

}
#endif
```

pybo_amd/csrc/gpx_internal.h:

```cpp
#pragma once
#include <hip/hip_runtime.h>
#include <stdint.h>
#include <string>
#include <vector>

#include "../../include/gpx.h"
#include "prune_hint.h"

namespace gpx {

constexpr int NB = 128;
constexpr int TBH = 128;
constexpr int DMAX = 1024;
constexpr int DMAX_RFF = DMAX;
constexpr int DMAX_RFF_RESIDENT = 64;
constexpr int TOPK_MAX = 4096;
constexpr int TOPK_PASS = 64;
constexpr int PEND_MAX = 8;

enum Timer {
    T_GRAM = 0, T_CHOL, T_TRTRI, T_ALPHA, T_XGRAM, T_TRMM, T_ACQ, T_RFF, T_NLAUNCH, T_FLOP, T_COPY, T_APPEND,
    T_RANK1, T_RFFSWEEP, T_RFFOPS, T_TGFALL, T_SCLK, T_RFFCLK, T_AHEAD, T_BOUND, T_BATCH, T_JOINT, T_COUNT
};

// ... 1 lines not shown

struct EnsBatchMember {
    const double *cq, *cp, *invell;
    double *qp, *V, *cross, *scal, *xs;
    double rho, bias, sn2;
};

}

struct CholGraphKey {
    int64_t Np;
    int w, rl, merge, fuse;
    const void *S, *R, *T, *U, *flag;
    hipStream_t s2, s3, s4;
};

struct gpx_handle {
    int device = 0;
    hipStream_t stream = nullptr;
    bool own_stream = false;
    hipStream_t stream2 = nullptr;
    hipStream_t stream3 = nullptr;
    hipStream_t stream4 = nullptr;
    hipEvent_t ev_chain = nullptr, ev_far = nullptr, ev_rest = nullptr;
    hipEvent_t ev_row[8] = {nullptr, nullptr, nullptr, nullptr, nullptr, nullptr, nullptr, nullptr};
    int x_skip = 0;
    int x_bg = 0, x_bg_lds = 72, x_bg_iters = 10000;
    hipStream_t stream_bg = nullptr;
    int chol_merge = 1;
    int chol_fuse = 0;
    int chol_graph = 0;
    hipGraphExec_t chol_exec = nullptr;
    CholGraphKey chol_key;
    int chol_rl = 1;
    int chol_w = 0;
    int chol_tg = 1;
    int tg_min = 2;
    int tg_max = 160;
    int tg_chunks = 0;
    int tg_nap = 0;
    int tg_db = -1;
    int tg_fuse = 1;
    int tg_db_max = 112;
    int tg_grid = 0;
    int tg_isolate = -1;
    int tg_trace = 0;
    int tg_tmo_ms = 0;
    bool tg_launched = false;
    int tg_fallbacks = 0;
    void* tg = nullptr;
    std::string err;

    bool fitted = false;
    int stage = 0;
    int ahead_top = 0;
    bool want_ahead = false;
    int trtri_ahead = 1;
    int trtri_ahead_min = 8;
    bool diag_inv_pending = false;
    bool eager_inverse = false;
    int grad_form = 0;
    int grad_rb_cs = 0;
    int grad_kernel = -1;
    int trtri_left = 0;
    bool refine_inverse = false;
    double* drefine = nullptr;
    int64_t cap_refine = 0;
    int64_t N = 0, Np = 0, d = 0;
    int kernel_id = 0;
    double rho = 1, sn2 = 0, bias = 0;
    std::vector<double> ell;
    int64_t fail_pivot = -1;

    int64_t cap_np = 0, cap_d = 0;
    double* dXs = nullptr;
    double* dXraw = nullptr;
    double* dy = nullptr;
    double* dS = nullptr;
    double* dR = nullptr;
    double* dT = nullptr;
    double* dU = nullptr;
    double* da = nullptr;
    double* dalpha = nullptr;
    double* dinvell = nullptr;
    double* hinv = nullptr;
    hipEvent_t ev_inv = nullptr;
    bool inv_inflight = false;
    double* hpin = nullptr;
    int64_t cap_hpin = 0;
    double* hpin_dev = nullptr;
    char* dsmall = nullptr;
    unsigned long long* dclk = nullptr;
    int* dflag = nullptr;
    double* dscal = nullptr;

    int64_t chunk = 0;
    int super_m = 8;
    int tile_order = -1;
    int64_t cap_ks = 0;
    double* dKs = nullptr;
    double* dQp = nullptr;
    double* dPp = nullptr;
    int64_t cap_part = 0;
    double* dXc = nullptr;
    int64_t cap_xc = 0;
    double* dout = nullptr;
    int64_t cap_out = 0;
    double* dblkv = nullptr;
    int64_t* dblki = nullptr;
    int64_t cap_blk = 0;
    int64_t cap_blki = 0;
    double* dtopv = nullptr;
    int64_t* dtopi = nullptr;
    int64_t cap_top = 0;
    const double* last_topv = nullptr;
    const int64_t* last_topi = nullptr;
    int64_t last_topn = 0;
    double* drff = nullptr;
    int64_t cap_rff = 0;
    double* drffs = nullptr;
    int64_t cap_rffs = 0;
    double* dgrad = nullptr;
    int64_t cap_grad = 0;
    double* dens = nullptr;
    int64_t cap_ens = 0;
    int prune = -1;
    char* dprune = nullptr;
    int64_t cap_prune = 0;
    struct SelectRecord {
        int path = -1;
        int64_t M = 0, k = 0, G = 0, Gg = 0, done = 0, cap = 0, nsurv = 0;
        double gate = 0.0;
        bool hinted = false;
        const double* ub = nullptr;
        const int64_t* idx = nullptr;
        const double* sc = nullptr;
    };
    struct PruneRecord : SelectRecord {
        const int* st = nullptr;
        int bound_kernel = -1;
        bool kept = false;
        int nR = 0;
        int64_t nsurv2 = 0;
        const double *qR = nullptr, *ub2 = nullptr;
        const int64_t* idx2 = nullptr;
    } prune_rec;
    struct EnsPruneRecord : SelectRecord {
        int n = 0;
        const double* delta = nullptr;
    } ens_rec;
    gpx::PruneHint prune_hint, ens_hint;
    int prune_keep = 0;
    int prune_bound = -1;
    int prune_rows = -1;
    int short_map = -1;
    char* dkeep = nullptr;
    int64_t cap_keep = 0;

    const double* app_w = nullptr;
    bool cache_on = false;
    bool cache_valid = false;
    int64_t cache_M = 0;
    double* dcZ = nullptr;
    double* dcq = nullptr;
    double* dcp = nullptr;
    int64_t cap_cz = 0, cap_cq = 0;
    double* dpend = nullptr;
    int64_t pend_ld = 0;
    int npend = 0;

    bool spec_active = false;
    bool spec_launched = false;
    bool spec_used = false;
    bool apply_pending = false;
    uint64_t gen = 0, spec_gen = 0;
    std::vector<double> spec_x;
    double* dspec = nullptr;
    int64_t cap_spec = 0, spec_ld = 0, spec_M = 0;
    hipEvent_t ev_spec_go = nullptr, ev_spec_done = nullptr;

    double* dbsel = nullptr;
    int64_t cap_bsel = 0;
    std::vector<gpx::EnsBatchMember> bsel_desc;

    double* djoint = nullptr;
    int64_t cap_joint = 0;

    double* dkg = nullptr;
    int64_t cap_kg = 0;
    double* dkgw = nullptr;
    int64_t cap_kgw = 0;
    std::vector<double> kg_A;
    uint64_t kg_gen = 0;
    int64_t kg_Np = 0;

    double* dbatch = nullptr;
    int64_t cap_batch = 0;
    double* dhyper = nullptr;
    int64_t cap_hyper = 0;

    std::vector<gpx::EventPair> pending;
    std::vector<hipEvent_t> pool;
    double tacc[gpx::T_COUNT] = {0};
};

namespace gpx {

void launch_scale_x(hipStream_t s, const double* X, int64_t n, int64_t np, int d, const double* invell,
                    double* Xs);
void launch_gram_sym(hipStream_t s, const double* Xs, int64_t N, int64_t Np, int d, int kernel_id,
                     double rho, double sn2, double* S);
int ensure_side_streams(gpx_handle* h);
void launch_cholesky(gpx_handle* h);
bool launch_cholesky_tg(gpx_handle* h);
int tg_abort_code(gpx_handle* h);
int64_t tg_trace_copy(gpx_handle* h, long long* out, int64_t n);
void tg_free(gpx_handle* h);
int64_t tg_tasks_copy(int nP, int chunks, int16_t* out, int64_t cap, int64_t* counts);
void launch_trtri(gpx_handle* h);
void launch_trtri_ahead(gpx_handle* h, hipStream_t s, int top);
int trtri_top(int nP);
void launch_refine_inverse(gpx_handle* h, double* tmp);
void launch_alpha(gpx_handle* h);
void launch_kinv_diag(gpx_handle* h, double* out);
void launch_transpose_lower(hipStream_t s, const double* R, int64_t Np, double* out, int64_t N);
void launch_cholesky_small(hipStream_t s, double* S, double* R, int64_t np, int* flag);
void launch_posterior_wide(hipStream_t s, const double* A, const double* v, const double* z, int n, int64_t np, double sc,
                           double sn2, double* B, double* R, double* work, int* flag, double* theta);

void launch_cross_gram(hipStream_t s, const double* Xs, int64_t rows, int64_t N, int d, const double* Xc,
                       int64_t m0, int64_t M, int64_t cols, const double* invell, int kernel_id,
                       double rho, double* Ks, int64_t ldk);
void launch_sweep_trmm(hipStream_t s, const double* U, int64_t Np, int nR, const double* Ks, int64_t ldk,
                       int64_t cols, const double* a, double* Qp, double* Pp, int64_t ldp,
                       int tile_order, int super_m, unsigned long long* clk, int short_map = -1);
void launch_acq(hipStream_t s, const double* Qp, const double* Pp, int64_t ldp, int nrb, int64_t m0,
                int64_t cols_valid, double rho, double bias, int acq_id, double p0, double* acq_out,
                double* mu_out, double* s2_out, double* qsum, double* psum);
struct MesArg;
void launch_acq_mes(hipStream_t s, const double* Qp, const double* Pp, int64_t ldp, int nrb, int64_t m0,
                    int64_t cols_valid, double rho, double bias, const MesArg& ys, double* acq_out,
                    double* mu_out, double* s2_out, double* qsum, double* psum);
void launch_kg_solve(hipStream_t s, const double* U, int64_t Np, int64_t N, int m, const double* V, double* W);
void launch_kg_cross(hipStream_t s, const double* B, int64_t Np, const double* Ks, int64_t ldk, int64_t cols, double* C, int64_t ldc);
void launch_acq_kg(hipStream_t s, const double* Qp, const double* Pp, int64_t ldp, int nrb, int64_t m0, int64_t cols_valid,
                   double rho, double bias, double sn2, int kid, int d, const double* X, const double* invell, const double* As, int m,
                   const double* al, const double* C, int64_t ldc, double* acq_out, double* mu_out, double* s2_out, double* qsum,
                   double* psum);
void launch_kg_point_sums(hipStream_t s, const double* Xs, int64_t N, int d, const double* Z, int np, const double* invell, int kid,
                          double rho, const double* B, const double* alpha, const double* Wz, const double* Vz, double* S);
void launch_kg_point_final(hipStream_t s, const double* S, int np, int d, const double* Z, const double* invell, const double* As,
                           int m, const double* al, int kid, double rho, double bias, double sn2, double* L, double* f, double* g);
void launch_pend_store(hipStream_t s, const double* w, int64_t Nj, int64_t ldw, const double* scal, double* row,
                       double* pscal_j);
void launch_cache_apply(hipStream_t s, const double* v, const double* scal, int64_t M, double* qsum, double* psum);
void launch_scale_point(hipStream_t s, const double* x, const double* invell, int d, double* xs);
void launch_sweep_rank1_v(hipStream_t s, const double* Xs, int64_t Ntot, int d, const double* Wq, int64_t ldw,
                          const double* pscal, const double* Z, int64_t M, const double* invell, int kernel_id,
                          double rho, const double* xlast, double* vout, const double* skip = nullptr);
void launch_sweep_rankq(hipStream_t s, const double* Xs, int64_t Ntot, int d, const double* Wq, int64_t ldw, int q,
                        const double* pscal, const double* Z, int64_t M, const double* invell, int kernel_id,
                        double rho, double* qsum, double* psum);
void launch_topk(hipStream_t s, const double* vals, int64_t M, int k, double* blkv, int64_t* blki,
                 int64_t nblk, double* topv, int64_t* topi);
void launch_topk_merge(hipStream_t s, double* vals, int64_t* idx, int64_t n, int k, double* topv, int64_t* topi);
void launch_topk_rows(hipStream_t s, const double* vals, int64_t M, int64_t S, int k, double* blkv, int64_t* blki,
                      int64_t nblk, double* topv, int64_t* topi);
int64_t topk_blocks(int64_t M);
void launch_prune_alpha(hipStream_t s, const double* U, int64_t Np, const double* a, double rho, double bias, double* alpha2,
                        double* sabs, double* sc);
constexpr int BM_SC_RX2 = 6, BM_SC_RZ2 = 7, BM_SC_GUARD = 8, BM_SC_USE = 9;
constexpr int BM_SC_E32 = 10, BM_SC_BADW = 11, BM_SC_USE32 = 12, BM_SC_FAC32 = 13, BM_SC_FLUSH32 = 14;
int bound_mfma_ks(int kernel_id, int d);
int64_t bound_mfma_ws_words(int64_t Np);
void launch_bound_mfma(hipStream_t s, const double* Xs, int64_t N, int64_t Np, int d, const double* alpha2, double rho,
                       const double* Z, int64_t M, const double* invell, int force, bool allow32, double* ws, double* sc, double* out);
void launch_bound_mfma32(hipStream_t s, const float* A32, const float* W32, const float* NX32, int KS, bool nc, int ntile, int d,
                         const double* Z, int64_t M, const double* invell, const double* cen, const double* sc, double* out);
void launch_prune_ub(hipStream_t s, const double* dots, double* ub, int64_t M, int64_t skip, const double* sc, double rho,
                     double bias, double p0);
void launch_prune_ub2(hipStream_t s, const double* Qp, int64_t ldp, int nR, int64_t j0, int64_t cols_valid, const int64_t* idx,
                      const double* dots, const double* sc, double rho, double bias, double p0, double* ub2, double* qR_out);
void launch_sel_remap(hipStream_t s, const int64_t* idx, int64_t* idx2, int64_t n);
void launch_prune_ub_fold(hipStream_t s, const double* dots, double* acc, int64_t M, const double* sc, double rho, double bias,
                          double p0, int first, double* delta_out);
void launch_prune_ub_mean(hipStream_t s, double* acc, int64_t M, int64_t skip, double n);
void launch_prune_mean(hipStream_t s, const double* v, int64_t n, double* out);
void launch_sel_threshold(hipStream_t s, const double* v, int64_t M, int G, int* hist, int* st);
int64_t sel_blocks(int64_t M);
void launch_sel_compact(hipStream_t s, const double* v, int64_t M, int mode, const int* st, const double* tau, int64_t* blk,
                        int64_t cap, const double* Xc, int d, int64_t* idx, double* Xg, double* tau_seen = nullptr);
void launch_sel_scatter(hipStream_t s, const int64_t* idx, const double* vals, int64_t n, double* out, double* mark);
void launch_fill_neg_inf(hipStream_t s, double* out, int64_t from, int64_t M);

int ensemble_predict_grad_host(gpx_handle* const* mem, int n, const double* Xc, int64_t M, double* mu, double* s2,
                               double* dmu, double* ds2);
int predict_mean_host(gpx_handle* h, const double* Xc, int64_t M, double* mu, double* dmu);
int predict_grad_host(gpx_handle* h, const double* Xc, int64_t M, double* mu, double* s2, double* dmu,
                      double* ds2);

int ensure_inverse(gpx_handle* h);

int loglik_host(gpx_handle* h, double* out);
void launch_loglik(gpx_handle* h, double* out);
int loglik_grad_host(gpx_handle* h, double* loglik, double* grad);
int loglik_batch_host(gpx_handle* h, int64_t B, const double* hyp, double* out);
int append_host(gpx_handle* h, const double* x, double ynew);
int grow_factor_if_full(gpx_handle* h);
void launch_append_prepare(gpx_handle* h, hipStream_t s, const double* dx, double* dks, double* dg, double* dr,
                           double* dtu, double resid, double* scal, int* flag);
struct SpecBuf { double *x, *xs, *ks, *g, *r, *tu, *row, *pscal, *scal, *v; };
SpecBuf spec_layout(const gpx_handle* h);
int rff_grad_host(gpx_handle* h, const double* W, const double* b, const double* theta, int64_t n, int64_t d,
                  double bias, const double* Xc, int64_t M, double* f, double* g);

int batch_blocks(int64_t M);
void launch_batch_score(hipStream_t s, int j, int64_t M, const double* cq, const double* cp, double* qp, double* V,
                        const double* cross, const double* scal, const unsigned char* taken, double rho, double bias,
                        int acq_id, double p0, double* s2_out, double* partv, int64_t* parti);
void launch_batch_pick(hipStream_t s, int j, int64_t M, int d, const double* partv, const int64_t* parti, const double* Z,
                       const double* invell, const double* qp, const double* V, double rho, double sn2, double* x,
                       double* xs, double* scal, double* cross, double* sel_val, int64_t* sel_idx, double* sel_s2,
                       unsigned char* taken);
void launch_ens_batch_score(hipStream_t s, int j, int n, int64_t M, const EnsBatchMember* mem, const unsigned char* taken,
                            int acq_id, double p0, double* partv, int64_t* parti);
void launch_ens_batch_pick(hipStream_t s, int j, int n, int64_t nb, int64_t M, int d, const double* partv, const int64_t* parti,
                           const double* Z, const EnsBatchMember* mem, double* x, double* sel_val, int64_t* sel_idx,
                           double* sel_s2, unsigned char* taken);
void launch_ens_same_grid(hipStream_t s, const double* Za, const double* Zb, int64_t words, int* flag);

void launch_cov_trmm(hipStream_t s, const double* U, int64_t Np, const double* Ks, int64_t cols, double* V);
void launch_cov_mu(hipStream_t s, const double* V, int64_t Np, int64_t cols, const double* a, double bias, double* Pp, double* mu);
void launch_cov_syrk(hipStream_t s, const double* V, int64_t Np, const double* Kss, int64_t Mp, double* C);
void launch_cov_form(hipStream_t s, const double* C, int64_t M, int64_t Mp, double add, double* B);
void launch_cov_draw(hipStream_t s, const double* R, int64_t Mp, int64_t M, const double* z, int64_t S, const double* mu,
                     const int* flag, double* out);

extern int g_rff_variant;
void launch_rff_mfma(hipStream_t s, const double* Wt, const double* bt, const double* tt, int S, int nfb, int n, int d,
                     int dp, double bias, const double* Xc, int64_t M, double* vals, unsigned long long* clk);
int64_t rff_gram_batch_scratch(int64_t S, int64_t Np);
void launch_rff_posterior(hipStream_t s, const double* A, const double* v, const double* z, int S, int n, double sc,
                          double sn2, double* theta, int* flag);
void launch_rff_gram_batch(hipStream_t s, const double* Xraw, int64_t N, int64_t Np, int d, int dp,
                           const double* Wt, const double* bt, int S, int n, const double* y, double bias,
                           double* scratch, double* A, double* v);
void launch_rff_gram(hipStream_t s, const double* Xraw, const double* Ft_scratch, int64_t N, int d,
                     const double* W, const double* b, int n, const double* y, double bias, double* A,
                     double* v);

void launch_ens_accum(hipStream_t s, double* acc0, double* acc1, const double* t0, const double* t1, int64_t M,
                      int mode, int first);
void launch_ens_finish(hipStream_t s, const double* acc0, const double* acc1, int64_t M, int mode, double n,
                       double beta, double* out, double* mu_out, double* s2_out);
void launch_grid_sobol(hipStream_t s, const uint32_t* sv, int bits, int64_t first, int64_t M, int d,
                       const double* bounds, double* X);
void launch_grid_uniform(hipStream_t s, uint64_t seed, int64_t first, int64_t M, int d, const double* bounds,
                         double* X);

}
```

pybo_amd/csrc/kernels_bound32.hip:

```cpp
#include <hip/hip_runtime.h>

#include "bound_f32.h"
#include "gpx_internal.h"
#include "gpx_math.h"

namespace gpx {

constexpr int BM32_XN = 128;

typedef float f4 __attribute__((ext_vector_type(4)));

template <int KS, bool NC>
__global__ __launch_bounds__(256, (KS + (NC ? 1 : 0) <= 4) ? 4 : 3) void k_bound_mfma32(const float* __restrict__ A, const float* __restrict__ W4,
                                                          const float* __restrict__ NX4, int ntile, int d, const double* __restrict__ Z,
                                                          int64_t M, const double* __restrict__ invell, const double* __restrict__ cen,
                                                          const double* __restrict__ sc, double* __restrict__ out) {
    __shared__ double redA[4][BM32_XN], redB[4][BM32_XN];
    if (sc[BM_SC_USE32] != 1.0) return;
    const int lane = threadIdx.x & 63, w = __builtin_amdgcn_readfirstlane(threadIdx.x >> 6);
    const int col = lane & 15, g = lane >> 4;
    const int64_t n0 = (int64_t)blockIdx.x * BM32_XN;
    float b[8][KS], nz[NC ? 8 : 1];
    unsigned lost = 0;
#pragma unroll
    for (int j = 0; j < 8; ++j) {
        const int64_t n = n0 + j * 16 + col;
#pragma unroll
        for (int ks = 0; ks < KS; ++ks) b[j][ks] = 0.0f;
        double n2 = 0.0;
        if (n < M) {
            for (int k = 0; k < d; ++k) {
                const double v = bound_zt(Z[n * d + k], invell[k], cen[k]);
                n2 = fma(v, v, n2);
#pragma unroll
                for (int ks = 0; ks < KS; ++ks) b[j][ks] = (k == 4 * ks + g) ? (float)v : b[j][ks];
            }
            if (!NC) {
#pragma unroll
                for (int ks = 0; ks < KS; ++ks) {
                    b[j][ks] = (d == 4 * ks + g) ? 1.0f : b[j][ks];
                    b[j][ks] = (d + 1 == 4 * ks + g) ? (float)(B32_LOG2E * (-0.5 * n2)) : b[j][ks];
                }
            }
        }
        if (NC) nz[j] = (float)(B32_LOG2E * (-0.5 * n2));
        lost |= (n2 < __builtin_huge_val()) ? 0u : (1u << j);
    }
    float accA[8], accB[8];
#pragma unroll
    for (int j = 0; j < 8; ++j) accA[j] = accB[j] = 0.0f;
    unsigned ao = ((unsigned)w * KS * 64 + lane) * 4, wo = ((unsigned)w * 16 + g * 4) * 4;
    const auto ld1 = [](const float* p, unsigned o) { return *reinterpret_cast<const float*>(reinterpret_cast<const char*>(p) + o); };
    const auto ld4 = [](const float* p, unsigned o) { return *reinterpret_cast<const f4*>(reinterpret_cast<const char*>(p) + o); };
    float a[KS], an[KS];
    f4 wv, wn, xv = {0.0f, 0.0f, 0.0f, 0.0f}, xn = {0.0f, 0.0f, 0.0f, 0.0f};
#pragma unroll
    for (int ks = 0; ks < KS; ++ks) an[ks] = ld1(A, ao + ks * 256);
    wn = ld4(W4, wo);
    if (NC) xn = ld4(NX4, wo);
#pragma unroll 1
    for (int t = w; t < ntile; t += 4) {
#pragma unroll
        for (int ks = 0; ks < KS; ++ks) a[ks] = an[ks];
        wv = wn;
        xv = xn;
        if (t + 4 < ntile) {
            ao += 4 * KS * 64 * 4;
            wo += 4 * 16 * 4;
#pragma unroll
            for (int ks = 0; ks < KS; ++ks) an[ks] = ld1(A, ao + ks * 256);
            wn = ld4(W4, wo);
            if (NC) xn = ld4(NX4, wo);
        }
        f4 wa;
#pragma unroll
        for (int r = 0; r < 4; ++r) wa[r] = __builtin_fabsf(wv[r]);
#pragma unroll
        for (int j = 0; j < 8; ++j) {
            f4 c = {0.0f, 0.0f, 0.0f, 0.0f};
            if (NC) {
#pragma unroll
                for (int r = 0; r < 4; ++r) c[r] = xv[r] + nz[j];
            }
#pragma unroll
            for (int ks = 0; ks < KS; ++ks) c = __builtin_amdgcn_mfma_f32_16x16x4f32(a[ks], b[j][ks], c, 0, 0, 0);
#pragma unroll
            for (int r = 0; r < 4; ++r) {
                const float k = __builtin_amdgcn_exp2f(c[r]);
                accA[j] = __builtin_fmaf(wv[r], k, accA[j]);
                accB[j] = __builtin_fmaf(wa[r], k, accB[j]);
            }
        }
    }
#pragma unroll
    for (int j = 0; j < 8; ++j) {
        double va = (double)accA[j], vb = (double)accB[j];
        va += __shfl_xor(va, 16);
        va += __shfl_xor(va, 32);
        vb += __shfl_xor(vb, 16);
        vb += __shfl_xor(vb, 32);
        if (g == 0) {
            redA[w][j * 16 + col] = ((lost >> j) & 1u) ? __builtin_nan("") : va;
            redB[w][j * 16 + col] = vb;
        }
    }
    __syncthreads();
    if (threadIdx.x < BM32_XN) {
        const int64_t n = n0 + threadIdx.x;
        const double sa = ((redA[0][threadIdx.x] + redA[1][threadIdx.x]) + redA[2][threadIdx.x]) + redA[3][threadIdx.x];
        const double sb = ((redB[0][threadIdx.x] + redB[1][threadIdx.x]) + redB[2][threadIdx.x]) + redB[3][threadIdx.x];
        if (n < M) out[n] = (sa != sa) ? sa : bound32_hi(sa, sb, sc[BM_SC_FAC32], sc[BM_SC_FLUSH32]);
    }
}

void launch_bound_mfma32(hipStream_t s, const float* A32, const float* W32, const float* NX32, int KS, bool nc, int ntile, int d,
                         const double* Z, int64_t M, const double* invell, const double* cen, const double* sc, double* out) {
    const dim3 grid((unsigned)((M + BM32_XN - 1) / BM32_XN));
#define GPX_BM32(K, C) hipLaunchKernelGGL((k_bound_mfma32<K, C>), grid, dim3(256), 0, s, A32, W32, NX32, ntile, d, Z, M, invell, cen, sc, out)
    switch (2 * KS + (nc ? 1 : 0)) {
        case 2: GPX_BM32(1, false); break;
        case 3: GPX_BM32(1, true); break;
        case 4: GPX_BM32(2, false); break;
        case 5: GPX_BM32(2, true); break;
        case 6: GPX_BM32(3, false); break;
        case 7: GPX_BM32(3, true); break;
        case 8: GPX_BM32(4, false); break;
        case 9: GPX_BM32(4, true); break;
        default: GPX_BM32(5, false); break;
    }
#undef GPX_BM32
}

}
```

pybo_amd/csrc/kernels_sweep.hip:

```cpp
#include "gemm_core.h"
#include "gpx_internal.h"
#include "gpx_math.h"
#include "bound_exp.h"
#include "bound_f32.h"
#include "sweep_map.h"

namespace gpx {

constexpr int XK = 64, XN = 128, XDC = 16;

template <bool FIRST>
__device__ __forceinline__ void dist_step(const double (*xo)[XK], const double (*xc)[XN], int k, int ty, int tx,
                                          double (&r2)[8][4]) {
    double a8[8], b4[4];
#pragma unroll
    for (int a = 0; a < 8; ++a) a8[a] = xo[k][ty * 8 + a];
#pragma unroll
    for (int b = 0; b < 4; ++b) b4[b] = xc[k][tx * 4 + b];
#pragma unroll
    for (int a = 0; a < 8; ++a)
#pragma unroll
        for (int b = 0; b < 4; ++b) {
            const double df = a8[a] - b4[b];
            r2[a][b] = FIRST ? df * df : fma(df, df, r2[a][b]);
// ... 556 lines not shown
    __shared__ double sv[4];
    __shared__ int64_t si[4];
    blkv += (int64_t)blockIdx.x * n;
    blki += (int64_t)blockIdx.x * n;
    topv += (int64_t)blockIdx.x * k;
    topi += (int64_t)blockIdx.x * k;
    for (int it = 0; it < k; ++it) {
        double bv = GPX_NEG_INF;
        int64_t bi = GPX_IDX_NONE;
        int64_t bpos = -1;
        for (int64_t e = threadIdx.x; e < n; e += 256) {
            const int64_t idx = blki[e];
            if (idx != GPX_IDX_NONE && better(blkv[e], idx, bv, bi)) { bv = blkv[e]; bi = idx; bpos = e; }
        }
        const int64_t mine = bi;
        block_argmax(bv, bi, sv, si);
        if (bi != GPX_IDX_NONE && mine == bi && bpos >= 0) blki[bpos] = GPX_IDX_NONE;
        if (threadIdx.x == 0) { topv[it] = bv; topi[it] = (bi == GPX_IDX_NONE) ? -1 : bi; }
        __syncthreads();
    }
}

void launch_topk_merge(hipStream_t s, double* vals, int64_t* idx, int64_t n, int k, double* topv, int64_t* topi) {
    hipLaunchKernelGGL(k_topk_merge, dim3(1), dim3(256), 0, s, vals, idx, n, k, topv, topi);
}

int64_t topk_blocks(int64_t M) { return (M + TK_PER_BLOCK - 1) / TK_PER_BLOCK; }

void launch_topk_rows(hipStream_t s, const double* vals, int64_t M, int64_t S, int k, double* blkv, int64_t* blki,
                      int64_t nblk, double* topv, int64_t* topi) {
    hipLaunchKernelGGL(k_topk_block, dim3((unsigned)nblk, (unsigned)S), dim3(256), 0, s, vals, M, k, blkv, blki,
                       (const double*)nullptr, (const int64_t*)nullptr);
    hipLaunchKernelGGL(k_topk_merge, dim3((unsigned)S), dim3(256), 0, s, blkv, blki, nblk * k, k, topv, topi);
}

void launch_topk(hipStream_t s, const double* vals, int64_t M, int k, double* blkv, int64_t* blki,
                 int64_t nblk, double* topv, int64_t* topi) {
    for (int done = 0; done < k; done += TOPK_PASS) {
        const int kk = (k - done < TOPK_PASS) ? k - done : TOPK_PASS;
        const double* cv = done ? topv + done - 1 : nullptr;
        const int64_t* ci = done ? topi + done - 1 : nullptr;
        hipLaunchKernelGGL(k_topk_block, dim3((unsigned)nblk), dim3(256), 0, s, vals, M, kk, blkv, blki, cv, ci);
        hipLaunchKernelGGL(k_topk_merge, dim3(1), dim3(256), 0, s, blkv, blki, nblk * kk, kk, topv + done, topi + done);
    }
}

constexpr double PRUNE_TAU_MIN = 1e-280;
constexpr double PRUNE_SLACK = 1e-6;

__global__ __launch_bounds__(256) void k_prune_alpha(const double* __restrict__ U, int64_t Np, const double* __restrict__ a,
                                                     double* __restrict__ alpha2, double* __restrict__ sabs) {
    __shared__ double r0[256], r1[256];
    const int64_t k = blockIdx.x;
    const double* row = U + k * Np;
    double s = 0.0, t = 0.0;
    for (int64_t m = k + threadIdx.x; m < Np; m += 256) {
        const double pr = row[m] * a[m];
        s += pr;
        t += fabs(pr);
    }
    r0[threadIdx.x] = s;
    r1[threadIdx.x] = t;
    __syncthreads();
    for (int w = 128; w > 0; w >>= 1) {
        if ((int)threadIdx.x < w) {
            r0[threadIdx.x] += r0[threadIdx.x + w];
            r1[threadIdx.x] += r1[threadIdx.x + w];
        }
        __syncthreads();
    }
    if (threadIdx.x == 0) {
        alpha2[k] = r0[0];
        sabs[k] = r1[0];
    }
}

__global__ __launch_bounds__(256) void k_prune_delta(const double* __restrict__ sabs, int64_t Np, double rho, double bias,
                                                     double* __restrict__ sc) {
    __shared__ double r0[256];
    double s = 0.0;
    for (int64_t m = threadIdx.x; m < Np; m += 256) s += sabs[m];
    r0[threadIdx.x] = s;
    __syncthreads();
    for (int w = 128; w > 0; w >>= 1) {
        if ((int)threadIdx.x < w) r0[threadIdx.x] += r0[threadIdx.x + w];
        __syncthreads();
    }
    if (threadIdx.x == 0) {
        sc[0] = r0[0];
        sc[1] = 8.0 * (double)(Np + 16) * 1.1102230246251565e-16 * fma(rho, r0[0], fabs(bias));
        sc[2] = -1.0;
        sc[3] = 0.0;
    }
}

void launch_prune_alpha(hipStream_t s, const double* U, int64_t Np, const double* a, double rho, double bias, double* alpha2,
                        double* sabs, double* sc) {
    hipLaunchKernelGGL(k_prune_alpha, dim3((unsigned)Np), dim3(256), 0, s, U, Np, a, alpha2, sabs);
    hipLaunchKernelGGL(k_prune_delta, dim3(1), dim3(256), 0, s, sabs, Np, rho, bias, sc);
}

constexpr int BM_KS_MAX = 5;
int bound_mfma_ks(int kernel_id, int d) { return (kernel_id == GPX_KERN_SE_ARD && d + 2 <= 4 * BM_KS_MAX) ? (d + 5) / 4 : 0; }

static bool bound_mfma_normc(int d) { return d > 0 && (d + 3) / 4 < (d + 5) / 4; }
static int bound_mfma_steps(int d) { return bound_mfma_normc(d) ? (d + 3) / 4 : (d + 5) / 4; }

__device__ __forceinline__ void block_max_nonneg(double v, double* slot, double* red) {
    red[threadIdx.x] = (v == v) ? v : 0.0;
    __syncthreads();
    for (int w = 128; w > 0; w >>= 1) {
        if ((int)threadIdx.x < w) red[threadIdx.x] = fmax(red[threadIdx.x], red[threadIdx.x + w]);
        __syncthreads();
    }
    if (threadIdx.x == 0)
        atomicMax(reinterpret_cast<unsigned long long*>(slot), (unsigned long long)__double_as_longlong(red[0]));
}

__global__ __launch_bounds__(256) void k_bound_centre(const double* __restrict__ Xs, int64_t N, int d, double* __restrict__ cen,
                                                      double* __restrict__ sc) {
    __shared__ double lo[256], hi[256];
    for (int k = 0; k < d; ++k) {
        double a = __builtin_huge_val(), b = -__builtin_huge_val();
        for (int64_t i = threadIdx.x; i < N; i += 256) {
            const double x = Xs[i * d + k];
            a = fmin(a, x);
            b = fmax(b, x);
        }
        lo[threadIdx.x] = a;
        hi[threadIdx.x] = b;
        __syncthreads();
        for (int w = 128; w > 0; w >>= 1) {
            if ((int)threadIdx.x < w) {
                lo[threadIdx.x] = fmin(lo[threadIdx.x], lo[threadIdx.x + w]);
                hi[threadIdx.x] = fmax(hi[threadIdx.x], hi[threadIdx.x + w]);
            }
            __syncthreads();
        }
        if (threadIdx.x == 0) cen[k] = 0.5 * lo[0] + 0.5 * hi[0];
        __syncthreads();
    }
    if (threadIdx.x == 0) {
        sc[BM_SC_RX2] = 0.0;
        sc[BM_SC_RZ2] = 0.0;
        sc[BM_SC_BADW] = 0.0;
    }
}

__global__ __launch_bounds__(256) void k_bound_aug(const double* __restrict__ Xs, int64_t N, int64_t Np, int d, int KS,
                                                   const double* __restrict__ cen, const double* __restrict__ alpha2, double rho,
                                                   double* __restrict__ A, double* __restrict__ W4, double* __restrict__ NX4,
                                                   float* __restrict__ A32, double* __restrict__ sc) {
    __shared__ double red[256];
    const int64_t i = (int64_t)blockIdx.x * 256 + threadIdx.x;
    double n2 = 0.0, badw = 0.0;
    if (i < Np) {
        const int64_t t = i >> 4;
        const int row = (int)(i & 15);
        double* At = A + t * KS * 64 + row;
        const bool live = i < N;
        for (int k = 0; k < 4 * KS; ++k) {
            double v = 0.0;
            if (live && k < d) {
                v = Xs[i * d + k] - cen[k];
                n2 = fma(v, v, n2);
            }
            if (live && !NX4 && k == d) v = -0.5 * n2;
            if (live && !NX4 && k == d + 1) v = 1.0;
            At[(k >> 2) * 64 + (k & 3) * 16] = v;
            if (A32) A32[t * KS * 64 + row + (k >> 2) * 64 + (k & 3) * 16] = (float)((live && k <= d) ? B32_LOG2E * v : v);
        }
        const int g = row & 3, r = row >> 2;
        const double wt = live ? rho * alpha2[i] : 0.0;
        W4[t * 16 + 4 * g + r] = wt;
        if (NX4) NX4[t * 16 + 4 * g + r] = live ? -0.5 * n2 : 0.0;
        if (A32) {
            float* W32 = A32 + Np * 4 * KS;
            W32[i] = (float)wt;
            if (NX4) W32[Np + i] = live ? (float)(B32_LOG2E * (-0.5 * n2)) : 0.0f;
            badw = bound32_bad_weight(wt);
        }
    }
    block_max_nonneg(n2, sc + BM_SC_RX2, red);
    if (A32) block_max_nonneg(badw, sc + BM_SC_BADW, red);
}

__global__ __launch_bounds__(256) void k_bound_rz(const double* __restrict__ Z, int64_t M, int d, const double* __restrict__ invell,
                                                  const double* __restrict__ cen, double* __restrict__ sc) {
    __shared__ double red[256];
    const int64_t n = (int64_t)blockIdx.x * 256 + threadIdx.x;
    double n2 = 0.0;
    if (n < M)
        for (int k = 0; k < d; ++k) {
            const double v = bound_zt(Z[n * d + k], invell[k], cen[k]);
            n2 = fma(v, v, n2);
        }
    block_max_nonneg(n2, sc + BM_SC_RZ2, red);
}

__global__ void k_bound_guard(int d, int64_t Np, int force, int want32, double rho, double* __restrict__ sc) {
    const double R = sqrt(sc[BM_SC_RX2]) + sqrt(sc[BM_SC_RZ2]);
    const double gv = (double)(d + 4) * R * R;
    const bool use64 = force > 0 || gv <= (double)Np;
    sc[BM_SC_GUARD] = gv;
    sc[BM_SC_USE] = use64 ? 1.0 : 0.0;
    double E = __builtin_nan(""), use32 = 0.0, fac = 0.0, fl = 0.0;
    if (want32) {
        E = bound32_E(d, (double)(Np / 16), gv);
        use32 = (force == 2 || (use64 && E <= B32_E_MAX && sc[BM_SC_BADW] == 0.0)) ? 1.0 : 0.0;
        fac = bound32_factor(E, sc[BM_SC_BADW]);
        fl = bound32_flush(rho * sc[0] * (1.0 + 0x1p-20), (double)Np);
    }
    sc[BM_SC_E32] = E;
    sc[BM_SC_USE32] = use32;
    sc[BM_SC_FAC32] = fac;
    sc[BM_SC_FLUSH32] = fl;
}

template <int KS, bool NC>
__global__ __launch_bounds__(256, (KS + (NC ? 1 : 0) <= 3) ? 4 : 3) void k_bound_mfma(const double* __restrict__ A, const double* __restrict__ W4,
                                                       const double* __restrict__ NX4, int ntile, int d, const double* __restrict__ Z,
                                                       int64_t M, const double* __restrict__ invell, const double* __restrict__ cen,
                                                       const double* __restrict__ sc, double* __restrict__ out) {
    __shared__ double red[4][XN];
    __shared__ double tab[BEXP_NT];
    if (sc[BM_SC_USE] != 1.0 || sc[BM_SC_USE32] == 1.0) return;
    if (threadIdx.x < BEXP_NT) tab[threadIdx.x] = kBoundExpTab[threadIdx.x];
    const int lane = threadIdx.x & 63, w = __builtin_amdgcn_readfirstlane(threadIdx.x >> 6);
    const int col = lane & 15, g = lane >> 4;
    const int64_t n0 = (int64_t)blockIdx.x * XN;
    double b[8][KS], nz[NC ? 8 : 1];
    unsigned lost = 0;
#pragma unroll
    for (int j = 0; j < 8; ++j) {
        const int64_t n = n0 + j * 16 + col;
#pragma unroll
        for (int ks = 0; ks < KS; ++ks) b[j][ks] = 0.0;
        double n2 = 0.0;
        if (n < M) {
            for (int k = 0; k < d; ++k) {
                const double v = bound_zt(Z[n * d + k], invell[k], cen[k]);
                n2 = fma(v, v, n2);
#pragma unroll
                for (int ks = 0; ks < KS; ++ks) b[j][ks] = (k == 4 * ks + g) ? v : b[j][ks];
            }
            if (!NC) {
#pragma unroll
                for (int ks = 0; ks < KS; ++ks) {
                    b[j][ks] = (d == 4 * ks + g) ? 1.0 : b[j][ks];
                    b[j][ks] = (d + 1 == 4 * ks + g) ? -0.5 * n2 : b[j][ks];
                }
            }
        }
        if (NC) nz[j] = -0.5 * n2;
        lost |= (n2 < __builtin_huge_val()) ? 0u : (1u << j);
    }
    __syncthreads();
    double acc[8];
#pragma unroll
    for (int j = 0; j < 8; ++j) acc[j] = 0.0;
    unsigned ao = ((unsigned)w * KS * 64 + lane) * 8, wo = ((unsigned)w * 16 + g * 4) * 8, xo = wo;
    const auto ld1 = [](const double* p, unsigned o) { return *reinterpret_cast<const double*>(reinterpret_cast<const char*>(p) + o); };
    const auto ld4 = [](const double* p, unsigned o) { return *reinterpret_cast<const d4*>(reinterpret_cast<const char*>(p) + o); };
    double a[KS], an[KS];
    d4 wv, wn = {0.0, 0.0, 0.0, 0.0}, xv = {0.0, 0.0, 0.0, 0.0};
#pragma unroll
    for (int ks = 0; ks < KS; ++ks) an[ks] = ld1(A, ao + ks * 512);
    if (NC)
        xv = ld4(NX4, xo);
    else
        wn = ld4(W4, wo);
#pragma unroll 1
    for (int t = w; t < ntile; t += 4) {
#pragma unroll
        for (int ks = 0; ks < KS; ++ks) a[ks] = an[ks];
        wv = NC ? ld4(W4, wo) : wn;
        wo += 4 * 16 * 8;
        if (t + 4 < ntile) {
            ao += 4 * KS * 64 * 8;
#pragma unroll
            for (int ks = 0; ks < KS; ++ks) an[ks] = ld1(A, ao + ks * 512);
            if (!NC) wn = ld4(W4, wo);
        }
#pragma unroll
        for (int j = 0; j < 8; ++j) {
            d4 c = {0.0, 0.0, 0.0, 0.0};
            if (NC) {
#pragma unroll
                for (int r = 0; r < 4; ++r) c[r] = xv[r] + nz[j];
                if (j == 7) {
                    xo += (t + 4 < ntile) ? 4 * 16 * 8 : 0;
                    xv = ld4(NX4, xo);
                }
            }
#pragma unroll
            for (int ks = 0; ks < KS; ++ks) c = __builtin_amdgcn_mfma_f64_16x16x4f64(a[ks], b[j][ks], c, 0, 0, 0);
#pragma unroll
            for (int r = 0; r < 4; ++r) acc[j] = fma(wv[r], bound_exp<false>(__builtin_fmin(c[r], 0.0), tab), acc[j]);
        }
    }
#pragma unroll
    for (int j = 0; j < 8; ++j) {
        double v = acc[j];
        v += __shfl_xor(v, 16);
        v += __shfl_xor(v, 32);
        if (g == 0) red[w][j * 16 + col] = ((lost >> j) & 1u) ? __builtin_nan("") : v;
    }
    __syncthreads();
    if (threadIdx.x < XN) {
        const int64_t n = n0 + threadIdx.x;
        if (n < M) out[n] = ((red[0][threadIdx.x] + red[1][threadIdx.x]) + red[2][threadIdx.x]) + red[3][threadIdx.x];
    }
}

int64_t bound_mfma_ws_words(int64_t Np) { return Np * 4 * BM_KS_MAX + Np + 4 * BM_KS_MAX + Np * 2 * BM_KS_MAX + Np; }

void launch_bound_mfma(hipStream_t s, const double* Xs, int64_t N, int64_t Np, int d, const double* alpha2, double rho,
                       const double* Z, int64_t M, const double* invell, int force, bool allow32, double* ws, double* sc, double* out) {
    const int KS = bound_mfma_steps(d);
    const bool nc = bound_mfma_normc(d);
    double* A = ws;
    double* W4 = A + Np * 4 * KS;
    double* NX4 = nc ? W4 + Np : nullptr;
    double* cen = ws + Np * 4 * BM_KS_MAX + Np;
    const bool want32 = force == 2 || (force < 0 && allow32);
    float* A32 = want32 ? reinterpret_cast<float*>(cen + 4 * BM_KS_MAX) : nullptr;
    const float* W32 = want32 ? A32 + Np * 4 * KS : nullptr;
    const float* NX32 = (want32 && nc) ? W32 + Np : nullptr;
    hipLaunchKernelGGL(k_bound_centre, dim3(1), dim3(256), 0, s, Xs, N, d, cen, sc);
    hipLaunchKernelGGL(k_bound_aug, dim3((unsigned)((Np + 255) / 256)), dim3(256), 0, s, Xs, N, Np, d, KS, cen, alpha2, rho, A, W4, NX4, A32, sc);
    hipLaunchKernelGGL(k_bound_rz, dim3((unsigned)((M + 255) / 256)), dim3(256), 0, s, Z, M, d, invell, cen, sc);
    hipLaunchKernelGGL(k_bound_guard, dim3(1), dim3(1), 0, s, d, Np, force, want32 ? 1 : 0, rho, sc);
    const dim3 grid((unsigned)((M + XN - 1) / XN));
    const int ntile = (int)(Np / 16);
#define GPX_BM(K, C) hipLaunchKernelGGL((k_bound_mfma<K, C>), grid, dim3(256), 0, s, A, W4, NX4, ntile, d, Z, M, invell, cen, sc, out)
    switch (2 * KS + (nc ? 1 : 0)) {
        case 2: GPX_BM(1, false); break;
        case 3: GPX_BM(1, true); break;
        case 4: GPX_BM(2, false); break;
        case 5: GPX_BM(2, true); break;
        case 6: GPX_BM(3, false); break;
        case 7: GPX_BM(3, true); break;
        case 8: GPX_BM(4, false); break;
        case 9: GPX_BM(4, true); break;
        default: GPX_BM(5, false); break;
    }
#undef GPX_BM
    if (!want32) return;
    launch_bound_mfma32(s, A32, W32, NX32, KS, nc, ntile, d, Z, M, invell, cen, sc, out);
}

__global__ __launch_bounds__(256) void k_prune_ub(const double* __restrict__ dots, double* __restrict__ ub, int64_t M, int64_t skip,
                                                  const double* __restrict__ sc, double rho, double bias, double p0) {
    const int64_t n = (int64_t)blockIdx.x * 256 + threadIdx.x;
    if (n >= M) return;
    ub[n] = (n < skip) ? GPX_NEG_INF : acq_value(GPX_ACQ_EI, (bias + dots[n]) + sc[1], rho, p0);
}

void launch_prune_ub(hipStream_t s, const double* dots, double* ub, int64_t M, int64_t skip, const double* sc, double rho,
                     double bias, double p0) {
    hipLaunchKernelGGL(k_prune_ub, dim3((unsigned)((M + 255) / 256)), dim3(256), 0, s, dots, ub, M, skip, sc, rho, bias, p0);
}

__global__ __launch_bounds__(256) void k_prune_ub2(const double* __restrict__ Qp, int64_t ldp, int nR, int64_t j0, int64_t cols_valid,
                                                   const int64_t* __restrict__ idx, const double* __restrict__ dots,
                                                   const double* __restrict__ sc, double rho, double bias, double p0,
                                                   double* __restrict__ ub2, double* __restrict__ qR_out) {
    const int64_t n = (int64_t)blockIdx.x * 256 + threadIdx.x;
    if (n >= cols_valid) return;
    double q = 0.0;
    for (int rb = 0; rb < nR; ++rb) q += Qp[(int64_t)rb * ldp + n];
    const double s2R = fmax(rho - q, 1e-100);
    ub2[j0 + n] = acq_value(GPX_ACQ_EI, (bias + dots[idx[j0 + n]]) + sc[1], s2R, p0);
    if (qR_out) qR_out[j0 + n] = q;
}

void launch_prune_ub2(hipStream_t s, const double* Qp, int64_t ldp, int nR, int64_t j0, int64_t cols_valid, const int64_t* idx,
                      const double* dots, const double* sc, double rho, double bias, double p0, double* ub2, double* qR_out) {
    hipLaunchKernelGGL(k_prune_ub2, dim3((unsigned)((cols_valid + 255) / 256)), dim3(256), 0, s, Qp, ldp, nR, j0, cols_valid, idx,
                       dots, sc, rho, bias, p0, ub2, qR_out);
}

__global__ __launch_bounds__(256) void k_sel_remap(const int64_t* __restrict__ idx, int64_t* __restrict__ idx2, int64_t n) {
    const int64_t j = (int64_t)blockIdx.x * 256 + threadIdx.x;
    if (j < n) idx2[j] = idx[idx2[j]];
}

void launch_sel_remap(hipStream_t s, const int64_t* idx, int64_t* idx2, int64_t n) {
    if (n <= 0) return;
    hipLaunchKernelGGL(k_sel_remap, dim3((unsigned)((n + 255) / 256)), dim3(256), 0, s, idx, idx2, n);
}

__device__ __forceinline__ double ens_fold(int first, double acc, double ub) {
#pragma clang fp contract(off)
    return first ? ub : acc + ub;
}
__device__ __forceinline__ double ens_mean(double acc, double n) {
#pragma clang fp contract(off)
    return acc / n;
}

__global__ __launch_bounds__(256) void k_prune_ub_fold(const double* __restrict__ dots, double* __restrict__ acc, int64_t M,
                                                       const double* __restrict__ sc, double rho, double bias, double p0, int first,
                                                       double* __restrict__ delta_out) {
    const int64_t n = (int64_t)blockIdx.x * 256 + threadIdx.x;
    if (n >= M) return;
    const double ub = acq_value(GPX_ACQ_EI, (bias + dots[n]) + sc[1], rho, p0);
    acc[n] = ens_fold(first, first ? 0.0 : acc[n], ub);
    if (n == 0) *delta_out = sc[1];
}

void launch_prune_ub_fold(hipStream_t s, const double* dots, double* acc, int64_t M, const double* sc, double rho, double bias,
                          double p0, int first, double* delta_out) {
    hipLaunchKernelGGL(k_prune_ub_fold, dim3((unsigned)((M + 255) / 256)), dim3(256), 0, s, dots, acc, M, sc, rho, bias, p0, first,
                       delta_out);
}

__global__ __launch_bounds__(256) void k_prune_ub_mean(double* __restrict__ acc, int64_t M, int64_t skip, double n) {
    const int64_t c = (int64_t)blockIdx.x * 256 + threadIdx.x;
    if (c >= M) return;
    acc[c] = (c < skip) ? GPX_NEG_INF : ens_mean(acc[c], n);
}

void launch_prune_ub_mean(hipStream_t s, double* acc, int64_t M, int64_t skip, double n) {
    hipLaunchKernelGGL(k_prune_ub_mean, dim3((unsigned)((M + 255) / 256)), dim3(256), 0, s, acc, M, skip, n);
}

__global__ __launch_bounds__(256) void k_prune_mean(const double* __restrict__ v, int64_t n, double* __restrict__ out) {
    __shared__ double r0[256];
    double s = 0.0;
    for (int64_t m = threadIdx.x; m < n; m += 256) s += v[m];
    r0[threadIdx.x] = s;
    __syncthreads();
    for (int w = 128; w > 0; w >>= 1) {
        if ((int)threadIdx.x < w) r0[threadIdx.x] += r0[threadIdx.x + w];
        __syncthreads();
    }
    if (threadIdx.x == 0) out[0] = r0[0] / (double)n;
}

void launch_prune_mean(hipStream_t s, const double* v, int64_t n, double* out) {
    hipLaunchKernelGGL(k_prune_mean, dim3(1), dim3(256), 0, s, v, n, out);
}

constexpr int SEL_BINS = 4096;
constexpr int SEL_PER_THREAD = 16;
constexpr int SEL_PER_BLOCK = 256 * SEL_PER_THREAD;
__device__ __forceinline__ unsigned sel_key24(double v) {
    unsigned long long b = (unsigned long long)__double_as_longlong(v);
    b ^= (b >> 63) ? ~0ull : 0x8000000000000000ull;
    return (unsigned)(b >> 40);
}

__global__ __launch_bounds__(256) void k_sel_hist(const double* __restrict__ v, int64_t M, int pass, const int* __restrict__ st,
                                                  int* __restrict__ hist) {
    __shared__ int lh[SEL_BINS];
    for (int b = threadIdx.x; b < SEL_BINS; b += 256) lh[b] = 0;
    __syncthreads();
    const unsigned hi = pass ? (unsigned)st[0] : 0u;
    const int64_t base = (int64_t)blockIdx.x * SEL_PER_BLOCK;
    for (int e = 0; e < SEL_PER_THREAD; ++e) {
        const int64_t n = base + e * 256 + threadIdx.x;
        if (n >= M) break;
        const unsigned key = sel_key24(v[n]);
        if (!pass) atomicAdd(&lh[key >> 12], 1);
        else if ((key >> 12) == hi) atomicAdd(&lh[key & 4095u], 1);
    }
    __syncthreads();
    for (int b = threadIdx.x; b < SEL_BINS; b += 256)
        if (lh[b]) atomicAdd(&hist[b], lh[b]);
}

__global__ __launch_bounds__(256) void k_sel_pick(const int* __restrict__ hist, int pass, int G, int* __restrict__ st) {
    __shared__ int ts[256];
    int s = 0;
    for (int j = 0; j < 16; ++j) s += hist[threadIdx.x * 16 + j];
    ts[threadIdx.x] = s;
    __syncthreads();
    if (threadIdx.x == 0) {
        const int need = pass ? G - st[1] : G;
        int cum = 0, t = 255;
        for (; t > 0; --t) {
            if (cum + ts[t] >= need) break;
            cum += ts[t];
        }
        int b = t * 16 + 15;
        for (; b > t * 16; --b) {
            if (cum + hist[b] >= need) break;
            cum += hist[b];
        }
        if (!pass) {
            st[0] = b;
            st[1] = cum;
        } else {
            st[2] = (st[0] << 12) | b;
        }
    }
}

void launch_sel_threshold(hipStream_t s, const double* v, int64_t M, int G, int* hist, int* st) {
    const unsigned nblk = (unsigned)((M + SEL_PER_BLOCK - 1) / SEL_PER_BLOCK);
    (void)hipMemsetAsync(hist, 0, 2 * SEL_BINS * sizeof(int), s);
    for (int pass = 0; pass < 2; ++pass) {
        hipLaunchKernelGGL(k_sel_hist, dim3(nblk), dim3(256), 0, s, v, M, pass, st, hist + pass * SEL_BINS);
        hipLaunchKernelGGL(k_sel_pick, dim3(1), dim3(256), 0, s, hist + pass * SEL_BINS, pass, G, st);
    }
}

constexpr int SEL_A_SHIFT = 40;
constexpr long long SEL_E_MASK = (1ll << SEL_A_SHIFT) - 1;
__device__ __forceinline__ long long sel_class(int mode, double v, unsigned thr, double cut) {
    if (mode == 0) {
        const unsigned key = sel_key24(v);
        return key > thr ? (1ll << SEL_A_SHIFT) : (key == thr ? 1ll : 0ll);
    }
    return !(v < cut) ? 1ll : 0ll;
}
__device__ __forceinline__ double sel_cut(int mode, const double* tau) {
    if (mode == 0) return 0.0;
    const double t = *tau;
    return (t >= PRUNE_TAU_MIN) ? t * (1.0 - PRUNE_SLACK) : GPX_NEG_INF;
}

__global__ __launch_bounds__(256) void k_sel_count(const double* __restrict__ v, int64_t M, int mode, const int* __restrict__ st,
                                                   const double* __restrict__ tau, int64_t* __restrict__ blk,
                                                   double* __restrict__ tau_seen) {
    __shared__ unsigned long long cnt;
    if (threadIdx.x == 0) cnt = 0;
    __syncthreads();
    const unsigned thr = (unsigned)st[2];
    const double cut = sel_cut(mode, tau);
    const int64_t base = (int64_t)blockIdx.x * SEL_PER_BLOCK + (int64_t)threadIdx.x * SEL_PER_THREAD;
    long long c = 0;
    for (int e = 0; e < SEL_PER_THREAD; ++e)
        if (base + e < M) c += sel_class(mode, v[base + e], thr, cut);
    if (c) atomicAdd(&cnt, (unsigned long long)c);
    __syncthreads();
    if (threadIdx.x == 0) {
        blk[blockIdx.x] = (int64_t)cnt;
        if (tau_seen && blockIdx.x == 0) *tau_seen = *tau;
    }
}

__global__ __launch_bounds__(256) void k_sel_scan(int64_t* __restrict__ blk, int64_t nblk) {
    __shared__ int64_t sh[256];
    __shared__ int64_t carry;
    if (threadIdx.x == 0) carry = 0;
    __syncthreads();
    for (int64_t b0 = 0; b0 < nblk; b0 += 256) {
        const int64_t i = b0 + threadIdx.x;
        const int64_t mine = (i < nblk) ? blk[i] : 0;
        sh[threadIdx.x] = mine;
        __syncthreads();
        for (int w = 1; w < 256; w <<= 1) {
            const int64_t add = ((int)threadIdx.x >= w) ? sh[threadIdx.x - w] : 0;
            __syncthreads();
            sh[threadIdx.x] += add;
            __syncthreads();
        }
        if (i < nblk) blk[i] = carry + sh[threadIdx.x] - mine;
        __syncthreads();
        if (threadIdx.x == 255) carry += sh[255];
        __syncthreads();
    }
    if (threadIdx.x == 0) blk[nblk] = carry;
}

__global__ __launch_bounds__(256) void k_sel_write(const double* __restrict__ v, int64_t M, int mode, const int* __restrict__ st,
// ... 76 lines not shown
```

Measured before the change: 80.33.

## Add factorised fp32 bound walk with sign-partitioned weight rows

The fp32 matrix-pipe bound kernel gains a factorised variant that folds each observation's norm term into a precomputed weight (WF32). This drops the augmented norm column. Rows are reordered so positive weights come first, followed by zero padding and then the rest, and the kernel accumulates positive and other tiles separately instead of keeping both signed and absolute-weight accumulators. The aim is to cut per-tile exp/FMA work and register pressure in the pruning bound. In exchange it adds guard logic for exponent overflow and per-wave occupancy tuning. It also adds diagnostic reporting of the factorised flag and the tile split position.

```diff
diff --git a/pybo_amd/_lib.py b/pybo_amd/_lib.py
--- a/pybo_amd/_lib.py
+++ b/pybo_amd/_lib.py
@@ -734,11 +734,13 @@
     PRUNE_PATHS = ('plain', 'gate declined', 'pruned', 'fell back')
 
     def prune_report(self, vectors=True):
-        scal = np.full(20, np.nan)
+        scal = np.full(22, np.nan)
         self._check(self._lib.gpx_prune_report(self._h, _ptr(scal), len(scal), None, None, 0, None, None, 0))
         names = ('path', 'M', 'k', 'G', 'Gg', 'done', 'cap', 'nsurv', 'S', 'delta', 'tau', 'gate_s2', 'thr_key', 'kept',
-                 'bound_kernel', 'guard', 'nR', 'nsurv2', 'E', 'gate_hint')
+                 'bound_kernel', 'guard', 'nR', 'nsurv2', 'E', 'gate_hint', 'bound_fact', 'bound_tpos')
         r = dict(zip(names, scal.tolist()))
+        r['bound_fact'] = None if np.isnan(r['bound_fact']) else r['bound_fact'] == 1.0
+        r['bound_tpos'] = None if np.isnan(r['bound_tpos']) else int(r['bound_tpos'])
         r['gate_hint'] = r['gate_hint'] == 1.0
         r['bound_kernel'] = None if np.isnan(r['bound_kernel']) else ('generic', 'mfma', 'mfma32')[int(r['bound_kernel'])]
         for n in ('path', 'M', 'k', 'G', 'Gg', 'done', 'cap', 'nsurv', 'kept', 'nR', 'nsurv2'):
@@ -765,7 +767,7 @@
     def ensemble_prune_report(engines, vectors=True):
         lead = engines[0]
         handles = (_P * len(engines))(*[e._h for e in engines])
-        scal = np.full(11 + len(engines), np.nan)
+        scal = np.full(11 + 2 * len(engines), np.nan)
         lead._check(lead._lib.gpx_ensemble_prune_report(handles, len(engines), _ptr(scal), len(scal), None, None, 0))
         names = ('path', 'M', 'k', 'G', 'Gg', 'done', 'cap', 'nsurv', 'tau', 'gate')
         r = dict(zip(names, scal[:10].tolist()))
@@ -774,6 +776,7 @@
         r['path'] = Engine.PRUNE_PATHS[r['path']]
         r['delta'] = scal[10:10 + len(engines)].copy()
         r['gate_hint'] = scal[10 + len(engines)] == 1.0
+        r['bound_fact'] = scal[11 + len(engines):11 + 2 * len(engines)].copy()
         if vectors and r['path'] in ('pruned', 'fell back'):
             nidx = r['nsurv'] if r['path'] == 'pruned' else 0
             r['ub'] = np.empty(r['M'])
diff --git a/pybo_amd/csrc/api.hip b/pybo_amd/csrc/api.hip
--- a/pybo_amd/csrc/api.hip
+++ b/pybo_amd/csrc/api.hip
@@ -142,6 +142,7 @@
     {"prune", SHIP, -1, 1, "prune must be -1 (by size and gate), 0 (never) or 1 (wherever legal)", store<&gpx_handle::prune>},
     {"prune_keep", DIAG, 0, 1, "prune_keep must be 0 or 1", store<&gpx_handle::prune_keep>},
     {"prune_bound", DIAG, -1, 2, "prune_bound must be -1 (by guard), 0 (generic kernel), 1 (matrix-pipe kernel) or 2 (fp32 matrix-pipe kernel)", store<&gpx_handle::prune_bound>},
+    {"bound_fact", DIAG, 0, 1, "bound_fact must be 0 (the fp32 bound kernel never takes its factorised form) or 1 (by its guard)", store<&gpx_handle::bound_fact>},
     {"prune_rows", DIAG, -1, 1000000, "prune_rows must be -1 (by size), 0 (no second bound) or a number of block rows", store<&gpx_handle::prune_rows>},
     {"short_map", DIAG, -1, 1, "short_map must be -1 (by size), 0 (never) or 1 (wherever tile map 3 is in use)", store<&gpx_handle::short_map>},
     {"chol_w", SHIP, 0, 8, "chol_w must be 0 (by size) or in [2, 8]", store<&gpx_handle::chol_w>, [](int64_t v) { return v != 1; }},
@@ -385,7 +386,7 @@
             return fail(h, GPX_ESTATE, "prune_report: the last sweep ran without the option prune_keep");
         HIPCHK(h, hipSetDevice(h->device));
         HIPCHK(h, hipStreamSynchronize(h->stream));
-        double sc[16];
+        double sc[BM_SC_WORDS];
         int st[4] = {0, 0, 0, 0};
         for (double& v : sc) v = NAN;
         if (bound) {
@@ -393,13 +394,16 @@
             HIPCHK(h, hipMemcpy(st, r.st, sizeof st, hipMemcpyDeviceToHost));
         }
         const bool guarded_bound = bound && r.bound_kernel < 0;
-        double out[20];
+        double out[22];
         report_head(r, out);
         const double tail[12] = {sc[0], sc[1], sc[5], r.gate, bound ? (double)st[2] : NAN, r.kept ? 1.0 : 0.0,
                                  bound ? (guarded_bound ? sc[9] + sc[12] : 0.0) : NAN, guarded_bound ? sc[8] : NAN,
                                  (double)r.nR, (double)r.nsurv2, guarded_bound ? sc[10] : NAN, r.hinted ? 1.0 : 0.0};
         std::copy(tail, tail + 12, out + 8);
-        for (int i = 0; i < nscal && i < 20; ++i) scal[i] = out[i];
+        const bool f32 = guarded_bound && sc[BM_SC_USE32] == 1.0;
+        out[20] = f32 ? sc[BM_SC_FACT32] : NAN;
+        out[21] = f32 ? sc[BM_SC_TPOS32] : NAN;
+        for (int i = 0; i < nscal && i < 22; ++i) scal[i] = out[i];
         int rc;
         if ((rc = report_vectors(h, r, ub, idx, cap_idx))) return rc;
         if (ub_kept) HIPCHK(h, hipMemcpy(ub_kept, h->dkeep, (size_t)r.M * 8, hipMemcpyDeviceToHost));
@@ -1066,7 +1070,7 @@
 static int prune_ws(gpx_handle* h, int64_t M, int64_t cap, int64_t Gg, int64_t extra, PruneWs& w, bool rows = false) {
     const int64_t Np = h->Np;
     w.nsel = sel_blocks(M);
-    const int64_t words0 = M + cap + cap * h->d + cap + (w.nsel + 1) + 2 * Np + Gg + 16 + extra + (2 * 4096 + 8) / 2;
+    const int64_t words0 = M + cap + cap * h->d + cap + (w.nsel + 1) + 2 * Np + Gg + BM_SC_WORDS + extra + (2 * 4096 + 8) / 2;
     const int64_t words1 = (words0 + 3) / 4 * 4 + bound_mfma_ws_words(Np);
     const int64_t words = words1 + (rows ? M + 3 * cap + cap * h->d + sel_blocks(cap) + 1 : 0);
     if (!h->dprune || words * 8 > h->cap_prune) h->ens_rec = gpx_handle::EnsPruneRecord();
@@ -1081,7 +1085,7 @@
     w.sabs = w.alpha2 + Np;
     w.gs2 = w.sabs + Np;
     w.sc = w.gs2 + Gg;
-    w.extra = w.sc + 16;
+    w.extra = w.sc + BM_SC_WORDS;
     w.hist = reinterpret_cast<int*>(w.extra + extra);
     w.st = w.hist + 2 * 4096;
     w.bws = w.ub + (words0 + 3) / 4 * 4;
@@ -1102,8 +1106,8 @@
     hipStream_t s = h->stream;
     launch_prune_alpha(s, h->dU, h->Np, h->da, h->rho, h->bias, w.alpha2, w.sabs, w.sc);
     if (bound_mfma)
-        launch_bound_mfma(s, h->dXs, h->N, h->Np, (int)h->d, w.alpha2, h->rho, dXc, M, h->dinvell, h->prune_bound, M >= BOUND_F32_MIN_M, w.bws,
-                          w.sc, out);
+        launch_bound_mfma(s, h->dXs, h->N, h->Np, (int)h->d, w.alpha2, h->rho, dXc, M, h->dinvell, h->prune_bound, M >= BOUND_F32_MIN_M, h->bound_fact != 0,
+                          w.bws, w.sc, out);
     launch_sweep_rank1_v(s, h->dXs, h->N, (int)h->d, w.alpha2, h->Np, w.sc + 2, dXc, M, h->dinvell, h->kernel_id, h->rho,
                          nullptr, out, bound_mfma ? w.sc + 9 : nullptr);
 }
@@ -2047,8 +2051,10 @@
             }
             {
                 Span sp(h, T_BOUND);
-                bound_dots(h, dXc, M, wm, h->prune_bound != 0 && bound_mfma_ks(h->kernel_id, (int)h->d) > 0, t1);
-                launch_prune_ub_fold(h->stream, t1, ub, M, wm.sc, h->rho, h->bias, params[0], m == 0, delta + m);
+                const bool bound_mfma = h->prune_bound != 0 && bound_mfma_ks(h->kernel_id, (int)h->d) > 0;
+                bound_dots(h, dXc, M, wm, bound_mfma, t1);
+                launch_prune_ub_fold(h->stream, t1, ub, M, wm.sc, h->rho, h->bias, params[0], m == 0, delta + m,
+                                     bound_mfma ? 1 : 0, delta + n + m);
             }
             HIPCHK(L, hipStreamSynchronize(h->stream));
         }
@@ -2061,7 +2067,7 @@
     };
     ops.after_seeds = [&]() -> int { HIPCHK(L, hipStreamSynchronize(s)); return GPX_OK; };
     int64_t done = 0;
-    if ((rc = select_topk_pruned(L, members_ok, !d_out && !d_mu && !d_s2, acq_id, n, nPmax, Np_min, dXc, M, k, 2 * n, false, w, L->ens_hint, rec,
+    if ((rc = select_topk_pruned(L, members_ok, !d_out && !d_mu && !d_s2, acq_id, n, nPmax, Np_min, dXc, M, k, 3 * n, false, w, L->ens_hint, rec,
                                  out, ops, &done)))
         return rc;
     if ((rc = plain_rest(ops, dXc, done, sweep_chunk(L, M), M, out, d_mu, d_s2))) return rc;
@@ -2219,15 +2225,16 @@
         if ((ub || idx) && !bound) return fail(h, GPX_ESTATE, "ensemble_prune_report: the last ensemble sweep did not reach its bound pass");
         HIPCHK(h, hipSetDevice(h->device));
         HIPCHK(h, hipStreamSynchronize(h->stream));
-        std::vector<double> out((size_t)(11 + n_members), NAN);
+        std::vector<double> out((size_t)(11 + 2 * n_members), NAN);
         out[10 + n_members] = r.hinted ? 1.0 : 0.0;
         report_head(r, out.data());
         out[9] = r.gate;
         if (bound) {
             HIPCHK(h, hipMemcpy(&out[8], r.sc + 5, 8, hipMemcpyDeviceToHost));
             HIPCHK(h, hipMemcpy(&out[10], r.delta, (size_t)n_members * 8, hipMemcpyDeviceToHost));
-        }
-        for (int i = 0; i < nscal && i < 11 + n_members; ++i) scal[i] = out[i];
+            HIPCHK(h, hipMemcpy(&out[11 + n_members], r.delta + n_members, (size_t)n_members * 8, hipMemcpyDeviceToHost));
+        }
+        for (int i = 0; i < nscal && i < 11 + 2 * n_members; ++i) scal[i] = out[i];
         return report_vectors(h, r, ub, idx, cap_idx);
     });
 }
diff --git a/pybo_amd/csrc/bound_f32.h b/pybo_amd/csrc/bound_f32.h
--- a/pybo_amd/csrc/bound_f32.h
+++ b/pybo_amd/csrc/bound_f32.h
@@ -35,6 +35,23 @@
 
 GPX_B32_FN double bound32_flush(double sum_w, double Np) { return 0x1p-124 * (sum_w + Np); }
 
+constexpr int B32_ZROWS = 16;
+GPX_B32_FN long long bound32_row_dest(int sgn, long long rank, long long npos, long long nzero) {
+    return sgn > 0 ? rank : (sgn == 0 ? npos + B32_ZROWS + rank : npos + B32_ZROWS + nzero + rank);
+}
+GPX_B32_FN long long bound32_tpos(long long npos) { return (npos + 15) / 16; }
+
+constexpr double B32_FACT_XMAX = 120.0, B32_FACT_SMAX = 126.0;
+GPX_B32_FN double bound32_norm_factor(double n2) { return std::exp2(B32_LOG2E * (-0.5 * n2)); }
+GPX_B32_FN double bound32_bad_weight_fact(double w, double wp) {
+    const double a = std::fabs(wp);
+    return (w == 0.0 || (a >= B32_W_MIN && a <= B32_W_MAX)) ? 0.0 : 1.0;
+}
+GPX_B32_FN double bound32_fact_ok(double rx2, double rz2, double sum_w) {
+    const double X = B32_LOG2E * std::sqrt(rx2) * std::sqrt(rz2) * (1.0 + 0x1p-10);
+    return (X <= B32_FACT_XMAX && X + std::log2(sum_w) <= B32_FACT_SMAX) ? 1.0 : 0.0;
+}
+
 GPX_B32_FN double bound32_hi(double A, double B, double factor, double F) {
     if (!(factor < HUGE_VAL)) return (A != A || B != B) ? A + B : HUGE_VAL;
     const double m = factor * B + F;
diff --git a/pybo_amd/csrc/gpx_internal.h b/pybo_amd/csrc/gpx_internal.h
--- a/pybo_amd/csrc/gpx_internal.h
+++ b/pybo_amd/csrc/gpx_internal.h
@@ -177,6 +177,11 @@
     gpx::PruneHint prune_hint, ens_hint;
     int prune_keep = 0;
     int prune_bound = -1;
+#ifdef GPX_BOUND32_NOFACT
+    int bound_fact = 0;
+#else
+    int bound_fact = 1;
+#endif
     int prune_rows = -1;
     int short_map = -1;
     char* dkeep = nullptr;
@@ -295,12 +300,14 @@
 void launch_prune_alpha(hipStream_t s, const double* U, int64_t Np, const double* a, double rho, double bias, double* alpha2,
                         double* sabs, double* sc);
 constexpr int BM_SC_RX2 = 6, BM_SC_RZ2 = 7, BM_SC_GUARD = 8, BM_SC_USE = 9;
-constexpr int BM_SC_E32 = 10, BM_SC_BADW = 11, BM_SC_USE32 = 12, BM_SC_FAC32 = 13, BM_SC_FLUSH32 = 14;
+constexpr int BM_SC_E32 = 10, BM_SC_BADW = 11, BM_SC_USE32 = 12, BM_SC_FAC32 = 13, BM_SC_FLUSH32 = 14, BM_SC_TPOS32 = 15, BM_SC_FACT32 = 16;
+constexpr int BM_SC_WORDS = 20;
 int bound_mfma_ks(int kernel_id, int d);
 int64_t bound_mfma_ws_words(int64_t Np);
 void launch_bound_mfma(hipStream_t s, const double* Xs, int64_t N, int64_t Np, int d, const double* alpha2, double rho,
-                       const double* Z, int64_t M, const double* invell, int force, bool allow32, double* ws, double* sc, double* out);
-void launch_bound_mfma32(hipStream_t s, const float* A32, const float* W32, const float* NX32, int KS, bool nc, int ntile, int d,
+                       const double* Z, int64_t M, const double* invell, int force, bool allow32, bool allow_fact, double* ws, double* sc,
+                       double* out);
+void launch_bound_mfma32(hipStream_t s, const float* A32, const float* W32, const float* WF32, const float* NX32, int KS, bool nc, int ntile, int d,
                          const double* Z, int64_t M, const double* invell, const double* cen, const double* sc, double* out);
 void launch_prune_ub(hipStream_t s, const double* dots, double* ub, int64_t M, int64_t skip, const double* sc, double rho,
                      double bias, double p0);
@@ -308,7 +315,7 @@
                       const double* dots, const double* sc, double rho, double bias, double p0, double* ub2, double* qR_out);
 void launch_sel_remap(hipStream_t s, const int64_t* idx, int64_t* idx2, int64_t n);
 void launch_prune_ub_fold(hipStream_t s, const double* dots, double* acc, int64_t M, const double* sc, double rho, double bias,
-                          double p0, int first, double* delta_out);
+                          double p0, int first, double* delta_out, int guarded, double* fact_out);
 void launch_prune_ub_mean(hipStream_t s, double* acc, int64_t M, int64_t skip, double n);
 void launch_prune_mean(hipStream_t s, const double* v, int64_t n, double* out);
 void launch_sel_threshold(hipStream_t s, const double* v, int64_t M, int G, int* hist, int* st);
diff --git a/pybo_amd/csrc/kernels_bound32.hip b/pybo_amd/csrc/kernels_bound32.hip
--- a/pybo_amd/csrc/kernels_bound32.hip
+++ b/pybo_amd/csrc/kernels_bound32.hip
@@ -10,13 +10,17 @@
 
 typedef float f4 __attribute__((ext_vector_type(4)));
 
-template <int KS, bool NC>
-__global__ __launch_bounds__(256, (KS + (NC ? 1 : 0) <= 4) ? 4 : 3) void k_bound_mfma32(const float* __restrict__ A, const float* __restrict__ W4,
+constexpr int bm32_waves(int KS, bool NC) { return NC ? (KS <= 2 ? 5 : 4) : (KS == 1 ? 8 : (KS == 4 ? 4 : (KS == 5 ? 5 : 7))); }
+
+template <int KS, bool NC, bool FACT>
+__global__ __launch_bounds__(256, bm32_waves(KS, NC)) void k_bound_mfma32(const float* __restrict__ A, const float* __restrict__ W4,
                                                           const float* __restrict__ NX4, int ntile, int d, const double* __restrict__ Z,
                                                           int64_t M, const double* __restrict__ invell, const double* __restrict__ cen,
                                                           const double* __restrict__ sc, double* __restrict__ out) {
+    static_assert(!(FACT && NC), "the factorised walk reads no norms");
     __shared__ double redA[4][BM32_XN], redB[4][BM32_XN];
-    if (sc[BM_SC_USE32] != 1.0) return;
+    if (sc[BM_SC_USE32] != 1.0 || (sc[BM_SC_FACT32] == 1.0) != FACT) return;
+    const int tpos = (int)sc[BM_SC_TPOS32];
     const int lane = threadIdx.x & 63, w = __builtin_amdgcn_readfirstlane(threadIdx.x >> 6);
     const int col = lane & 15, g = lane >> 4;
     const int64_t n0 = (int64_t)blockIdx.x * BM32_XN;
@@ -35,7 +39,7 @@
 #pragma unroll
                 for (int ks = 0; ks < KS; ++ks) b[j][ks] = (k == 4 * ks + g) ? (float)v : b[j][ks];
             }
-            if (!NC) {
+            if (!NC && !FACT) {
 #pragma unroll
                 for (int ks = 0; ks < KS; ++ks) {
                     b[j][ks] = (d == 4 * ks + g) ? 1.0f : b[j][ks];
@@ -46,9 +50,9 @@
         if (NC) nz[j] = (float)(B32_LOG2E * (-0.5 * n2));
         lost |= (n2 < __builtin_huge_val()) ? 0u : (1u << j);
     }
-    float accA[8], accB[8];
+    float accP[8], accN[8];
 #pragma unroll
-    for (int j = 0; j < 8; ++j) accA[j] = accB[j] = 0.0f;
+    for (int j = 0; j < 8; ++j) accP[j] = accN[j] = 0.0f;
     unsigned ao = ((unsigned)w * KS * 64 + lane) * 4, wo = ((unsigned)w * 16 + g * 4) * 4;
     const auto ld1 = [](const float* p, unsigned o) { return *reinterpret_cast<const float*>(reinterpret_cast<const char*>(p) + o); };
     const auto ld4 = [](const float* p, unsigned o) { return *reinterpret_cast<const f4*>(reinterpret_cast<const char*>(p) + o); };
@@ -58,8 +62,7 @@
     for (int ks = 0; ks < KS; ++ks) an[ks] = ld1(A, ao + ks * 256);
     wn = ld4(W4, wo);
     if (NC) xn = ld4(NX4, wo);
-#pragma unroll 1
-    for (int t = w; t < ntile; t += 4) {
+    const auto tile = [&](float (&acc)[8], int t) {
 #pragma unroll
         for (int ks = 0; ks < KS; ++ks) a[ks] = an[ks];
         wv = wn;
@@ -72,9 +75,6 @@
             wn = ld4(W4, wo);
             if (NC) xn = ld4(NX4, wo);
         }
-        f4 wa;
-#pragma unroll
-        for (int r = 0; r < 4; ++r) wa[r] = __builtin_fabsf(wv[r]);
 #pragma unroll
         for (int j = 0; j < 8; ++j) {
             f4 c = {0.0f, 0.0f, 0.0f, 0.0f};
@@ -85,16 +85,17 @@
 #pragma unroll
             for (int ks = 0; ks < KS; ++ks) c = __builtin_amdgcn_mfma_f32_16x16x4f32(a[ks], b[j][ks], c, 0, 0, 0);
 #pragma unroll
-            for (int r = 0; r < 4; ++r) {
-                const float k = __builtin_amdgcn_exp2f(c[r]);
-                accA[j] = __builtin_fmaf(wv[r], k, accA[j]);
-                accB[j] = __builtin_fmaf(wa[r], k, accB[j]);
-            }
+            for (int r = 0; r < 4; ++r) acc[j] = __builtin_fmaf(wv[r], __builtin_amdgcn_exp2f(c[r]), acc[j]);
         }
-    }
+    };
+    int t = w;
+#pragma unroll 1
+    for (; t < tpos; t += 4) tile(accP, t);
+#pragma unroll 1
+    for (; t < ntile; t += 4) tile(accN, t);
 #pragma unroll
     for (int j = 0; j < 8; ++j) {
-        double va = (double)accA[j], vb = (double)accB[j];
+        double va = (double)accP[j] + (double)accN[j], vb = (double)accP[j] - (double)accN[j];
         va += __shfl_xor(va, 16);
         va += __shfl_xor(va, 32);
         vb += __shfl_xor(vb, 16);
@@ -107,16 +108,27 @@
     __syncthreads();
     if (threadIdx.x < BM32_XN) {
         const int64_t n = n0 + threadIdx.x;
-        const double sa = ((redA[0][threadIdx.x] + redA[1][threadIdx.x]) + redA[2][threadIdx.x]) + redA[3][threadIdx.x];
-        const double sb = ((redB[0][threadIdx.x] + redB[1][threadIdx.x]) + redB[2][threadIdx.x]) + redB[3][threadIdx.x];
+        double sa = ((redA[0][threadIdx.x] + redA[1][threadIdx.x]) + redA[2][threadIdx.x]) + redA[3][threadIdx.x];
+        double sb = ((redB[0][threadIdx.x] + redB[1][threadIdx.x]) + redB[2][threadIdx.x]) + redB[3][threadIdx.x];
+        if (FACT) {
+            double n2 = 0.0;
+            if (n < M)
+                for (int k = 0; k < d; ++k) {
+                    const double v = bound_zt(Z[n * d + k], invell[k], cen[k]);
+                    n2 = fma(v, v, n2);
+                }
+            const double cz = bound32_norm_factor(n2);
+            sa *= cz;
+            sb *= cz;
+        }
         if (n < M) out[n] = (sa != sa) ? sa : bound32_hi(sa, sb, sc[BM_SC_FAC32], sc[BM_SC_FLUSH32]);
     }
 }
 
-void launch_bound_mfma32(hipStream_t s, const float* A32, const float* W32, const float* NX32, int KS, bool nc, int ntile, int d,
-                         const double* Z, int64_t M, const double* invell, const double* cen, const double* sc, double* out) {
+void launch_bound_mfma32(hipStream_t s, const float* A32, const float* W32, const float* WF32, const float* NX32, int KS, bool nc, int ntile,
+                         int d, const double* Z, int64_t M, const double* invell, const double* cen, const double* sc, double* out) {
     const dim3 grid((unsigned)((M + BM32_XN - 1) / BM32_XN));
-#define GPX_BM32(K, C) hipLaunchKernelGGL((k_bound_mfma32<K, C>), grid, dim3(256), 0, s, A32, W32, NX32, ntile, d, Z, M, invell, cen, sc, out)
+#define GPX_BM32(K, C) hipLaunchKernelGGL((k_bound_mfma32<K, C, false>), grid, dim3(256), 0, s, A32, W32, NX32, ntile, d, Z, M, invell, cen, sc, out)
     switch (2 * KS + (nc ? 1 : 0)) {
         case 2: GPX_BM32(1, false); break;
         case 3: GPX_BM32(1, true); break;
@@ -129,6 +141,15 @@
         default: GPX_BM32(5, false); break;
     }
 #undef GPX_BM32
+#define GPX_BM32F(K) hipLaunchKernelGGL((k_bound_mfma32<K, false, true>), grid, dim3(256), 0, s, A32, WF32, nullptr, ntile, d, Z, M, invell, cen, sc, out)
+    switch (KS) {
+        case 1: GPX_BM32F(1); break;
+        case 2: GPX_BM32F(2); break;
+        case 3: GPX_BM32F(3); break;
+        case 4: GPX_BM32F(4); break;
+        default: GPX_BM32F(5); break;
+    }
+#undef GPX_BM32F
 }
 
 }
diff --git a/pybo_amd/csrc/kernels_sweep.hip b/pybo_amd/csrc/kernels_sweep.hip
--- a/pybo_amd/csrc/kernels_sweep.hip
+++ b/pybo_amd/csrc/kernels_sweep.hip
@@ -732,11 +732,50 @@
                                                    double* __restrict__ A, double* __restrict__ W4, double* __restrict__ NX4,
                                                    float* __restrict__ A32, double* __restrict__ sc) {
     __shared__ double red[256];
+    __shared__ int cnt[4], wcnt[4][2];
     const int64_t i = (int64_t)blockIdx.x * 256 + threadIdx.x;
+    int64_t i32 = 0, npos = 0;
+    if (A32) {
+        if (threadIdx.x < 4) cnt[threadIdx.x] = 0;
+        __syncthreads();
+        const int64_t i0 = (int64_t)blockIdx.x * 256;
+        int c[4] = {0, 0, 0, 0};
+        for (int64_t j = threadIdx.x; j < Np; j += 256) {
+            const double wj = (j < N) ? rho * alpha2[j] : 0.0;
+            const int p = wj > 0.0 ? 1 : 0, z = (wj > 0.0 || wj < 0.0) ? 0 : 1;
+            c[0] += p;
+            c[1] += z;
+            c[2] += (j < i0) ? p : 0;
+            c[3] += (j < i0) ? z : 0;
+        }
+#pragma unroll
+        for (int q = 0; q < 4; ++q) {
+            for (int o = 32; o > 0; o >>= 1) c[q] += __shfl_xor(c[q], o);
+            if ((threadIdx.x & 63) == 0) atomicAdd(&cnt[q], c[q]);
+        }
+        const double wi = (i < N) ? rho * alpha2[i] : 0.0;
+        const bool in = i < Np, p = in && wi > 0.0, z = in && !(wi > 0.0 || wi < 0.0);
+        const unsigned long long bp = __ballot(p), bz = __ballot(z), below = (1ull << (threadIdx.x & 63)) - 1ull;
+        const int wv = threadIdx.x >> 6;
+        if ((threadIdx.x & 63) == 0) {
+            wcnt[wv][0] = __popcll(bp);
+            wcnt[wv][1] = __popcll(bz);
+        }
+        __syncthreads();
+        int rp = cnt[2] + __popcll(bp & below), rz = cnt[3] + __popcll(bz & below);
+        for (int q = 0; q < wv; ++q) {
+            rp += wcnt[q][0];
+            rz += wcnt[q][1];
+        }
+        npos = cnt[0];
+        const int64_t rn = i - rp - rz;
+        i32 = bound32_row_dest(p ? 1 : (z ? 0 : -1), p ? rp : (z ? rz : rn), npos, cnt[1]);
+        if (i == 0) sc[BM_SC_TPOS32] = (double)bound32_tpos(npos);
+    }
     double n2 = 0.0, badw = 0.0;
     if (i < Np) {
-        const int64_t t = i >> 4;
-        const int row = (int)(i & 15);
+        const int64_t t = i >> 4, t32 = i32 >> 4;
+        const int row = (int)(i & 15), row32 = (int)(i32 & 15);
         double* At = A + t * KS * 64 + row;
         const bool live = i < N;
         for (int k = 0; k < 4 * KS; ++k) {
@@ -748,17 +787,26 @@
             if (live && !NX4 && k == d) v = -0.5 * n2;
             if (live && !NX4 && k == d + 1) v = 1.0;
             At[(k >> 2) * 64 + (k & 3) * 16] = v;
-            if (A32) A32[t * KS * 64 + row + (k >> 2) * 64 + (k & 3) * 16] = (float)((live && k <= d) ? B32_LOG2E * v : v);
+            if (A32) A32[t32 * KS * 64 + row32 + (k >> 2) * 64 + (k & 3) * 16] = (float)((live && k <= d) ? B32_LOG2E * v : v);
         }
         const int g = row & 3, r = row >> 2;
         const double wt = live ? rho * alpha2[i] : 0.0;
         W4[t * 16 + 4 * g + r] = wt;
         if (NX4) NX4[t * 16 + 4 * g + r] = live ? -0.5 * n2 : 0.0;
         if (A32) {
-            float* W32 = A32 + Np * 4 * KS;
-            W32[i] = (float)wt;
-            if (NX4) W32[Np + i] = live ? (float)(B32_LOG2E * (-0.5 * n2)) : 0.0f;
-            badw = bound32_bad_weight(wt);
+            const int64_t Np32 = Np + B32_ZROWS;
+            float* W32 = A32 + Np32 * 4 * KS;
+            const double wf = wt * bound32_norm_factor(n2);
+            W32[i32] = (float)wt;
+            W32[Np32 + i32] = (float)wf;
+            if (NX4) W32[2 * Np32 + i32] = live ? (float)(B32_LOG2E * (-0.5 * n2)) : 0.0f;
+            badw = fmax(bound32_bad_weight(wt), 0.5 * bound32_bad_weight_fact(wt, wf));
+            if (i < B32_ZROWS) {
+                const int64_t e = npos + i;
+                for (int k = 0; k < 4 * KS; ++k) A32[(e >> 4) * KS * 64 + (e & 15) + (k >> 2) * 64 + (k & 3) * 16] = 0.0f;
+                W32[e] = W32[Np32 + e] = 0.0f;
+                if (NX4) W32[2 * Np32 + e] = 0.0f;
+            }
         }
     }
     block_max_nonneg(n2, sc + BM_SC_RX2, red);
@@ -778,22 +826,25 @@
     block_max_nonneg(n2, sc + BM_SC_RZ2, red);
 }
 
-__global__ void k_bound_guard(int d, int64_t Np, int force, int want32, double rho, double* __restrict__ sc) {
+__global__ void k_bound_guard(int d, int64_t Np, int force, int want32, int allow_fact, double rho, double* __restrict__ sc) {
     const double R = sqrt(sc[BM_SC_RX2]) + sqrt(sc[BM_SC_RZ2]);
     const double gv = (double)(d + 4) * R * R;
     const bool use64 = force > 0 || gv <= (double)Np;
     sc[BM_SC_GUARD] = gv;
     sc[BM_SC_USE] = use64 ? 1.0 : 0.0;
-    double E = __builtin_nan(""), use32 = 0.0, fac = 0.0, fl = 0.0;
+    double E = __builtin_nan(""), use32 = 0.0, fact = 0.0, fac = 0.0, fl = 0.0;
     if (want32) {
+        const double bw = sc[BM_SC_BADW], sum_w = rho * sc[0] * (1.0 + 0x1p-20);
         E = bound32_E(d, (double)(Np / 16), gv);
-        use32 = (force == 2 || (use64 && E <= B32_E_MAX && sc[BM_SC_BADW] == 0.0)) ? 1.0 : 0.0;
-        fac = bound32_factor(E, sc[BM_SC_BADW]);
-        fl = bound32_flush(rho * sc[0] * (1.0 + 0x1p-20), (double)Np);
+        use32 = (force == 2 || (use64 && E <= B32_E_MAX && bw != 1.0)) ? 1.0 : 0.0;
+        fact = (allow_fact && use32 == 1.0 && E <= B32_E_MAX && bw == 0.0) ? bound32_fact_ok(sc[BM_SC_RX2], sc[BM_SC_RZ2], sum_w) : 0.0;
+        fac = bound32_factor(E, bw == 1.0 ? 1.0 : 0.0);
+        fl = bound32_flush(sum_w, (double)Np);
     }
     sc[BM_SC_E32] = E;
     sc[BM_SC_USE32] = use32;
     sc[BM_SC_FAC32] = fac;
+    sc[BM_SC_FACT32] = fact;
     sc[BM_SC_FLUSH32] = fl;
 }
 
@@ -893,10 +944,11 @@
     }
 }
 
-int64_t bound_mfma_ws_words(int64_t Np) { return Np * 4 * BM_KS_MAX + Np + 4 * BM_KS_MAX + Np * 2 * BM_KS_MAX + Np; }
+int64_t bound_mfma_ws_words(int64_t Np) { return Np * 4 * BM_KS_MAX + Np + 4 * BM_KS_MAX + (Np + B32_ZROWS) * (2 * BM_KS_MAX + 2); }
 
 void launch_bound_mfma(hipStream_t s, const double* Xs, int64_t N, int64_t Np, int d, const double* alpha2, double rho,
-                       const double* Z, int64_t M, const double* invell, int force, bool allow32, double* ws, double* sc, double* out) {
+                       const double* Z, int64_t M, const double* invell, int force, bool allow32, bool allow_fact, double* ws, double* sc,
+                       double* out) {
     const int KS = bound_mfma_steps(d);
     const bool nc = bound_mfma_normc(d);
     double* A = ws;
@@ -905,12 +957,14 @@
     double* cen = ws + Np * 4 * BM_KS_MAX + Np;
     const bool want32 = force == 2 || (force < 0 && allow32);
     float* A32 = want32 ? reinterpret_cast<float*>(cen + 4 * BM_KS_MAX) : nullptr;
-    const float* W32 = want32 ? A32 + Np * 4 * KS : nullptr;
-    const float* NX32 = (want32 && nc) ? W32 + Np : nullptr;
+    const int64_t Np32 = Np + B32_ZROWS;
+    const float* W32 = want32 ? A32 + Np32 * 4 * KS : nullptr;
+    const float* WF32 = want32 ? W32 + Np32 : nullptr;
+    const float* NX32 = (want32 && nc) ? WF32 + Np32 : nullptr;
     hipLaunchKernelGGL(k_bound_centre, dim3(1), dim3(256), 0, s, Xs, N, d, cen, sc);
     hipLaunchKernelGGL(k_bound_aug, dim3((unsigned)((Np + 255) / 256)), dim3(256), 0, s, Xs, N, Np, d, KS, cen, alpha2, rho, A, W4, NX4, A32, sc);
     hipLaunchKernelGGL(k_bound_rz, dim3((unsigned)((M + 255) / 256)), dim3(256), 0, s, Z, M, d, invell, cen, sc);
-    hipLaunchKernelGGL(k_bound_guard, dim3(1), dim3(1), 0, s, d, Np, force, want32 ? 1 : 0, rho, sc);
+    hipLaunchKernelGGL(k_bound_guard, dim3(1), dim3(1), 0, s, d, Np, force, want32 ? 1 : 0, allow_fact ? 1 : 0, rho, sc);
     const dim3 grid((unsigned)((M + XN - 1) / XN));
     const int ntile = (int)(Np / 16);
 #define GPX_BM(K, C) hipLaunchKernelGGL((k_bound_mfma<K, C>), grid, dim3(256), 0, s, A, W4, NX4, ntile, d, Z, M, invell, cen, sc, out)
@@ -927,7 +981,7 @@
     }
 #undef GPX_BM
     if (!want32) return;
-    launch_bound_mfma32(s, A32, W32, NX32, KS, nc, ntile, d, Z, M, invell, cen, sc, out);
+    launch_bound_mfma32(s, A32, W32, WF32, NX32, KS, nc, (int)(Np32 / 16), d, Z, M, invell, cen, sc, out);
 }
 
 __global__ __launch_bounds__(256) void k_prune_ub(const double* __restrict__ dots, double* __restrict__ ub, int64_t M, int64_t skip,
@@ -982,18 +1036,21 @@
 
 __global__ __launch_bounds__(256) void k_prune_ub_fold(const double* __restrict__ dots, double* __restrict__ acc, int64_t M,
                                                        const double* __restrict__ sc, double rho, double bias, double p0, int first,
-                                                       double* __restrict__ delta_out) {
+                                                       double* __restrict__ delta_out, int guarded, double* __restrict__ fact_out) {
     const int64_t n = (int64_t)blockIdx.x * 256 + threadIdx.x;
     if (n >= M) return;
     const double ub = acq_value(GPX_ACQ_EI, (bias + dots[n]) + sc[1], rho, p0);
     acc[n] = ens_fold(first, first ? 0.0 : acc[n], ub);
-    if (n == 0) *delta_out = sc[1];
+    if (n == 0) {
+        *delta_out = sc[1];
+        *fact_out = guarded ? ((sc[BM_SC_USE32] == 1.0 && sc[BM_SC_FACT32] == 1.0) ? 1.0 : 0.0) : __builtin_nan("");
+    }
 }
 
 void launch_prune_ub_fold(hipStream_t s, const double* dots, double* acc, int64_t M, const double* sc, double rho, double bias,
-                          double p0, int first, double* delta_out) {
+                          double p0, int first, double* delta_out, int guarded, double* fact_out) {
     hipLaunchKernelGGL(k_prune_ub_fold, dim3((unsigned)((M + 255) / 256)), dim3(256), 0, s, dots, acc, M, sc, rho, bias, p0, first,
-                       delta_out);
+                       delta_out, guarded, fact_out);
 }
 
 __global__ __launch_bounds__(256) void k_prune_ub_mean(double* __restrict__ acc, int64_t M, int64_t skip, double n) {
```

New measurement: 83.28 (median of 6 runs). +3.7%, better.
